# williamfgc/ROCm-MPI

Measured on AMD Instinct MI355X. Metric: T_eff (GB/s) + weak-scaling eff., 2D diffusion 1000 steps at 1/2/4/8 MI355X, higher is better.
Workload: dtype fp64

## Files before the change

csrc/bindings/module.cpp:

```cpp
#include <pybind11/pybind11.h>
#include <pybind11/stl.h>

#include <cstdint>
#include <string>
#include <tuple>
#include <vector>

#include "rma/config.h"
#include "rma/comm.h"
#include "rma/common.h"
#include "rma/executor.h"
#include "rma/gather.h"
#include "rma/halo.h"
#include "rma/ipc.h"
#include "rma/kernels.h"
#include "rma/loopback.h"
#include "rma/p2p.h"
#include "rma/plan.h"
#include "rma/topology.h"
#include "rma/trace.h"

namespace py = pybind11;
using namespace rma;

namespace {

template <typename T>
T* P(uintptr_t p) {
  return reinterpret_cast<T*>(p);
}
stream_t S(uintptr_t s) { return reinterpret_cast<stream_t>(s); }

using Rect4 = std::tuple<int64_t, int64_t, int64_t, int64_t>;
using Coef4 = std::tuple<double, double, double, double>;
using Geom = std::tuple<int64_t, int64_t, int64_t, int64_t, double, double, double, double, int,
                        int>;

std::vector<Rect> to_rects(const std::vector<Rect4>& v) {
  std::vector<Rect> r;
  for (auto& t : v) r.push_back({std::get<0>(t), std::get<1>(t), std::get<2>(t), std::get<3>(t)});
  return r;
}
StencilCoef to_coef(const Coef4& c) {
  return {std::get<0>(c), std::get<1>(c), std::get<2>(c), std::get<3>(c)};
}
TileGeom to_geom(const Geom& g) {
  TileGeom t;
  std::tie(t.gx0, t.gy0, t.nxg, t.nyg, t.dx, t.dy, t.xoff, t.yoff, t.periodx, t.periody) = g;
  return t;
}
Rect4 from_rect(const Rect& r) { return {r.x0, r.x1, r.y0, r.y1}; }

using Box6 = std::tuple<int64_t, int64_t, int64_t, int64_t, int64_t, int64_t>;
using Coef5 = std::tuple<double, double, double, double, double>;
using Geom3 = std::tuple<int64_t, int64_t, int64_t, int64_t, int64_t, int64_t, double, double,
                         double, double, double, double, int, int,
                         int>;
std::vector<Box> to_boxes(const std::vector<Box6>& v) {
  std::vector<Box> b;
  for (auto& t : v)
    b.push_back({std::get<0>(t), std::get<1>(t), std::get<2>(t), std::get<3>(t), std::get<4>(t),
                 std::get<5>(t)});
  return b;
}
StencilCoef3 to_coef3(const Coef5& c) {
  return {std::get<0>(c), std::get<1>(c), std::get<2>(c), std::get<3>(c), std::get<4>(c)};
}
TileGeom3 to_geom3(const Geom3& g) {
  TileGeom3 t;
  std::tie(t.gx0, t.gy0, t.gz0, t.nxg, t.nyg, t.nzg, t.dx, t.dy, t.dz, t.xoff, t.yoff, t.zoff,
           t.periodx, t.periody, t.periodz) = g;
  return t;
}

using FieldT = std::tuple<uintptr_t, std::array<int64_t, 3>, int, std::array<int64_t, 3>,
                          std::array<int64_t, 3>>;
std::vector<HaloField> to_fields(const std::vector<FieldT>& v) {
  std::vector<HaloField> out;
  for (auto& t : v) {
    HaloField f;
    f.ptr = reinterpret_cast<void*>(std::get<0>(t));
    f.size = std::get<1>(t);
    f.elem_bytes = std::get<2>(t);
    f.ol = std::get<3>(t);
    f.hw = std::get<4>(t);
    out.push_back(f);
  }
  return out;
}

}

PYBIND11_MODULE(_C, m) {
  m.doc() = "rocm_mpi_amd native core (HIP kernels for gfx950, RCCL halo exchange, executor)";
  static py::exception<Error> exc(m, "NativeError", PyExc_RuntimeError);
  py::register_exception_translator([](std::exception_ptr p) {
    try {
      if (p) std::rethrow_exception(p);
    } catch (const Error& e) {
      exc(e.what());
    }
  });

  m.def("set_rank_for_errors", &set_rank_for_errors);
  m.def("rccl_version", &rccl_version);
  m.def("rccl_library", &rccl_library);
  m.def("device_pci_bus_id", &device_pci_bus_id, py::arg("device"));
  m.def(
      "stencil_strip_cells",
      [](int64_t nx, int vec) {
        StencilTuning t;
        t.vec = vec;
        return stencil_strip_cells(nx, t);
      },
      py::arg("nx"), py::arg("vec") = 2);

  m.def(
      "stencil_rects",
      [](uintptr_t T2, uintptr_t T, uintptr_t iCp, int64_t nx, int64_t ny,
         const std::vector<Rect4>& rects, const Coef4& coef, int chunk_rows, int nontemporal,
         int kernel, uintptr_t stream, bool gpu, int unroll, int vec, int xcd_remap) {
        auto r = to_rects(rects);
        StencilTuning tn;
        tn.chunk_rows = chunk_rows;
        tn.nontemporal = nontemporal;
        tn.kernel = kernel;
        tn.unroll = unroll;
        tn.vec = vec;
        tn.xcd_remap = xcd_remap;
        if (gpu)
          stencil_rects_gpu(P<double>(T2), P<const double>(T), P<const double>(iCp), nx, ny,
                            r.data(), (int)r.size(), to_coef(coef), tn, S(stream));
        else {
          py::gil_scoped_release nogil;
          stencil_rects_cpu(P<double>(T2), P<const double>(T), P<const double>(iCp), nx, ny,
                            r.data(), (int)r.size(), to_coef(coef));
        }
      },
      py::arg("T2"), py::arg("T"), py::arg("iCp"), py::arg("nx"), py::arg("ny"), py::arg("rects"),
      py::arg("coef"), py::arg("chunk_rows") = 4, py::arg("nontemporal") = 3,
      py::arg("kernel") = 0, py::arg("stream") = 0, py::arg("gpu") = true,
      py::arg("unroll") = 4, py::arg("vec") = 2, py::arg("xcd_remap") = -1);
  m.def(
      "stencil2_rects",
      [](uintptr_t T2, uintptr_t T, uintptr_t iCp, int64_t nx, int64_t ny,
         const std::vector<Rect4>& rects, const Coef4& coef, int chunk_rows, int nontemporal,
         uintptr_t stream, bool gpu, int unroll, int xcd_remap) {
        auto r = to_rects(rects);
        StencilTuning tn;
        tn.chunk_rows = chunk_rows;
        tn.nontemporal = nontemporal;
        tn.unroll = unroll;
        tn.xcd_remap = xcd_remap;
        if (gpu)
          stencil2_rects_gpu(P<double>(T2), P<const double>(T), P<const double>(iCp), nx, ny,
                             r.data(), (int)r.size(), to_coef(coef), tn, S(stream));
        else {
          py::gil_scoped_release nogil;
          stencil2_rects_cpu(P<double>(T2), P<const double>(T), P<const double>(iCp), nx, ny,
                             r.data(), (int)r.size(), to_coef(coef));
        }
      },
      py::arg("T2"), py::arg("T"), py::arg("iCp"), py::arg("nx"), py::arg("ny"), py::arg("rects"),
      py::arg("coef"), py::arg("chunk_rows") = 8, py::arg("nontemporal") = 3,
      py::arg("stream") = 0, py::arg("gpu") = true, py::arg("unroll") = 2,
      py::arg("xcd_remap") = -1);
  m.def(
      "stencilk_rects",
      [](int K, uintptr_t T2, uintptr_t T, uintptr_t iCp, int64_t nx, int64_t ny,
         const std::vector<Rect4>& rects, const Coef4& coef, int chunk_rows, int nontemporal,
         uintptr_t stream, bool gpu, int xcd_remap, int vec, int kernel, int stages, int cols,
         bool uniform, double uniform_value) {
        auto r = to_rects(rects);
        StencilTuning tn;
        tn.cols = cols;
        tn.uniform = uniform;
        tn.uniform_value = uniform_value;
        tn.chunk_rows = chunk_rows;
        tn.nontemporal = nontemporal;
        tn.xcd_remap = xcd_remap;
        tn.vec = vec;
        tn.kernel = kernel;
        tn.stages = stages;
        if (gpu)
          stencilk_rects_gpu(K, P<double>(T2), P<const double>(T), P<const double>(iCp), nx, ny,
                             r.data(), (int)r.size(), to_coef(coef), tn, S(stream));
        else {
          const bool f5 = (kernel >= 5 && kernel <= 9) || kernel == 12 || kernel == 22;
          py::gil_scoped_release nogil;
          if (f5)
            stencilk5_rects_cpu(K, P<double>(T2), P<const double>(T), P<const double>(iCp), nx,
                                ny, r.data(), (int)r.size(), to_coef(coef));
          else
            stencilk_rects_cpu(K, P<double>(T2), P<const double>(T), P<const double>(iCp), nx,
                               ny, r.data(), (int)r.size(), to_coef(coef));
        }
      },
      py::arg("K"), py::arg("T2"), py::arg("T"), py::arg("iCp"), py::arg("nx"), py::arg("ny"),
      py::arg("rects"), py::arg("coef"), py::arg("chunk_rows") = 16, py::arg("nontemporal") = 3,
      py::arg("stream") = 0, py::arg("gpu") = true, py::arg("xcd_remap") = -1,
      py::arg("vec") = 2, py::arg("kernel") = 0, py::arg("stages") = 0, py::arg("cols") = 0,
      py::arg("uniform") = false, py::arg("uniform_value") = 0.0);
  m.def(
      "stencil3d_boxes",
      [](uintptr_t T2, uintptr_t T, uintptr_t iCp, int64_t nx, int64_t ny, int64_t nz,
         const std::vector<Box6>& boxes, const Coef5& coef, int rows, int unroll, int vec,
         int nontemporal, int chunk_z, int xcd_remap, uintptr_t stream, bool gpu) {
        auto b = to_boxes(boxes);
        if (gpu) {
          Stencil3DTuning tn;
          tn.rows = rows;
          tn.unroll = unroll;
          tn.vec = vec;
          tn.nontemporal = nontemporal;
          tn.chunk_z = chunk_z;
          tn.xcd_remap = xcd_remap;
          stencil3d_boxes_gpu(P<double>(T2), P<const double>(T), P<const double>(iCp), nx, ny, nz,
                              b.data(), (int)b.size(), to_coef3(coef), tn, S(stream));
        } else {
          py::gil_scoped_release nogil;
          stencil3d_boxes_cpu(P<double>(T2), P<const double>(T), P<const double>(iCp), nx, ny, nz,
                              b.data(), (int)b.size(), to_coef3(coef));
        }
      },
      py::arg("T2"), py::arg("T"), py::arg("iCp"), py::arg("nx"), py::arg("ny"), py::arg("nz"),
      py::arg("boxes"), py::arg("coef"), py::arg("rows") = 4, py::arg("unroll") = 2,
      py::arg("vec") = 2, py::arg("nontemporal") = 3, py::arg("chunk_z") = 0,
      py::arg("xcd_remap") = 1, py::arg("stream") = 0, py::arg("gpu") = true);
  m.def("stencil3d_has", &stencil3d_has, py::arg("rows"), py::arg("unroll"));
  m.def("init_gaussian3d", [](uintptr_t T, int64_t nx, int64_t ny, int64_t nz, const Geom3& g,
                              double lx, double ly, double lz, uintptr_t stream, bool gpu) {
    if (gpu)
      init_gaussian3d_gpu(P<double>(T), nx, ny, nz, to_geom3(g), lx, ly, lz, S(stream));
    else
      init_gaussian3d_cpu(P<double>(T), nx, ny, nz, to_geom3(g), lx, ly, lz);
  });
  m.def("init_random3d", [](uintptr_t A, int64_t nx, int64_t ny, int64_t nz, const Geom3& g,
                            uint64_t seed, double lo, double hi, uintptr_t stream, bool gpu) {
    if (gpu)
      init_random3d_gpu(P<double>(A), nx, ny, nz, to_geom3(g), seed, lo, hi, S(stream));
    else
      init_random3d_cpu(P<double>(A), nx, ny, nz, to_geom3(g), seed, lo, hi);
  });
  m.def(
      "stream_copy",
      [](uintptr_t b, uintptr_t a, int64_t n, uintptr_t s, int nt, int blocks) {
        stream_copy_gpu(P<double>(b), P<const double>(a), n, nt, blocks, S(s));
      },
      py::arg("b"), py::arg("a"), py::arg("n"), py::arg("stream"), py::arg("nt") = 0,
      py::arg("blocks") = 0);
  m.def(
      "stream_triad",
      [](uintptr_t c, uintptr_t a, uintptr_t b, double x, int64_t n, uintptr_t s, int nt,
         int blocks) {
        stream_triad_gpu(P<double>(c), P<const double>(a), P<const double>(b), x, n, nt, blocks,
                         S(s));
      },
      py::arg("c"), py::arg("a"), py::arg("b"), py::arg("x"), py::arg("n"), py::arg("stream"),
      py::arg("nt") = 0, py::arg("blocks") = 0);

  m.def("flux", [](uintptr_t qx, uintptr_t qy, uintptr_t T, int64_t nx, int64_t ny, double mlam,
                   double rdx, double rdy, uintptr_t stream, bool gpu) {
    if (gpu)
      flux_gpu(P<double>(qx), P<double>(qy), P<const double>(T), nx, ny, mlam, rdx, rdy,
               S(stream));
    else
      flux_cpu(P<double>(qx), P<double>(qy), P<const double>(T), nx, ny, mlam, rdx, rdy);
  });
  m.def("residual", [](uintptr_t dTdt, uintptr_t qx, uintptr_t qy, uintptr_t iCp, int64_t nx,
                       int64_t ny, double rdx, double rdy, uintptr_t stream, bool gpu) {
    if (gpu)
      residual_gpu(P<double>(dTdt), P<const double>(qx), P<const double>(qy),
                   P<const double>(iCp), nx, ny, rdx, rdy, S(stream));
    else
      residual_cpu(P<double>(dTdt), P<const double>(qx), P<const double>(qy),
                   P<const double>(iCp), nx, ny, rdx, rdy);
  });
  m.def("update", [](uintptr_t T, uintptr_t dTdt, int64_t nx, int64_t ny, double dt,
                     uintptr_t stream, bool gpu) {
    if (gpu)
      update_gpu(P<double>(T), P<const double>(dTdt), nx, ny, dt, S(stream));
    else
      update_cpu(P<double>(T), P<const double>(dTdt), nx, ny, dt);
  });
  m.def("init_gaussian", [](uintptr_t T, int64_t nx, int64_t ny, const Geom& g, double lx,
                            double ly, uintptr_t stream, bool gpu) {
    if (gpu)
      init_gaussian_gpu(P<double>(T), nx, ny, to_geom(g), lx, ly, S(stream));
    else
      init_gaussian_cpu(P<double>(T), nx, ny, to_geom(g), lx, ly);
  });
  m.def("init_random", [](uintptr_t A, int64_t nx, int64_t ny, const Geom& g, uint64_t seed,
                          double lo, double hi, uintptr_t stream, bool gpu) {
    if (gpu)
      init_random_gpu(P<double>(A), nx, ny, to_geom(g), seed, lo, hi, S(stream));
    else
      init_random_cpu(P<double>(A), nx, ny, to_geom(g), seed, lo, hi);
  });
  m.def("fill", [](uintptr_t A, int64_t n, double v, uintptr_t stream) {
    fill_gpu(P<double>(A), n, v, S(stream));
  });
  m.def("copy2d", [](uintptr_t dst, int64_t dst_ld, uintptr_t src, int64_t src_ld, int64_t n_o,
                     int64_t n_k, int elem_bytes, uintptr_t stream, bool gpu) {
    if (gpu)
      copy2d_gpu(P<void>(dst), dst_ld, P<const void>(src), src_ld, n_o, n_k, elem_bytes,
                 S(stream));
    else
      copy2d_cpu(P<void>(dst), dst_ld, P<const void>(src), src_ld, n_o, n_k, elem_bytes);
  });
  m.def("copy2d_batch", [](const std::vector<std::tuple<uintptr_t, int64_t, uintptr_t, int64_t,
                                                        int64_t, int64_t>>& copies,
                           int elem_bytes, uintptr_t stream, bool gpu) {
    std::vector<Copy2d> c;
    for (const auto& t : copies)
      c.push_back({P<void>(std::get<0>(t)), std::get<1>(t), P<const void>(std::get<2>(t)),
                   std::get<3>(t), std::get<4>(t), std::get<5>(t)});
    if (gpu)
      copy2d_batch_gpu(c.data(), (int)c.size(), elem_bytes, S(stream));
    else
      copy2d_batch_cpu(c.data(), (int)c.size(), elem_bytes);
  });
  m.def("copy2d_batch_max", [] { return kCopy2dBatch; });
  m.def("copy_blocks", [](const std::vector<std::tuple<uintptr_t, uintptr_t, int64_t, int64_t,
                                                       int64_t, int64_t, int64_t, int64_t,
                                                       int64_t>>& blocks,
                          int elem_bytes, uintptr_t stream, bool gpu) {
    std::vector<BlockCopy> c;
    for (const auto& t : blocks)
      c.push_back({P<void>(std::get<0>(t)), P<const void>(std::get<1>(t)), std::get<2>(t),
                   std::get<3>(t), std::get<4>(t), std::get<5>(t), std::get<6>(t),
                   std::get<7>(t), std::get<8>(t)});
    if (gpu)
      copy_blocks_gpu(c.data(), (int64_t)c.size(), elem_bytes, S(stream));
    else
      copy_blocks_cpu(c.data(), (int64_t)c.size(), elem_bytes);
  });
  m.def("copy_blocks_max", [] { return kCopyBlocksBatch; });
  m.def(
      "gather_plan",
      [](const std::array<int, 3>& dims, const std::array<int64_t, 3>& size, int elem_bytes) {
        const GatherPlan p = plan_gather(dims, size, elem_bytes);
        py::dict d;
        d["nprocs"] = p.nprocs;
        d["size_g"] = p.size_g;
        d["row_pitch_g"] = p.row_pitch_g;
        d["plane_pitch_g"] = p.plane_pitch_g;
        d["block_elems"] = p.block_elems;
        d["coords"] = p.coords;
        d["offsets"] = p.offset;
        d["contiguous_in_global"] = p.contiguous_in_global;
        return d;
      },
      py::arg("dims"), py::arg("size"), py::arg("elem_bytes"));
  m.def(
      "flag_wait",
      [](uintptr_t flag, uint64_t want, double timeout_s, uintptr_t err, uint32_t code,
         uintptr_t stream) {
        flag_wait_gpu(P<const uint64_t>(flag), want, timeout_s, P<uint32_t>(err), code, S(stream));
      },
      py::call_guard<py::gil_scoped_release>());
  m.def(
      "flag_write",
      [](uintptr_t flag, uint64_t value, uintptr_t stream) {
        flag_write_gpu(P<uint64_t>(flag), value, S(stream));
      },
      py::call_guard<py::gil_scoped_release>());
  m.def("reduce_workspace_doubles", &reduce_workspace_doubles);
  m.def("reduce_gpu", [](uintptr_t A, int64_t n, int op, uintptr_t out, uintptr_t ws,
                         uintptr_t stream) {
    reduce_gpu(P<const double>(A), n, op, P<double>(out), P<double>(ws), S(stream));
  });
  m.def("reduce_cpu",
        [](uintptr_t A, int64_t n, int op) { return reduce_cpu(P<const double>(A), n, op); });
  m.def("diag_string", &diag_string);
  m.def("diag_value", [](const std::string& k) { return diag_value(k.c_str()); });
  m.def("env_double", &env_double);
  m.def("env_choice", &env_choice);
  m.def("field_stats_workspace_doubles", &field_stats_workspace_doubles);
  m.def("field_stats_gpu", [](uintptr_t A, int64_t n, uintptr_t out3, uintptr_t ws,
                              uintptr_t stream) {
    field_stats_gpu(P<const double>(A), n, P<double>(out3), P<double>(ws), S(stream));
  });
  m.def("field_stats_cpu", [](uintptr_t A, int64_t n) {
    double o[3];
    field_stats_cpu(P<const double>(A), n, o);
    return std::make_tuple(o[0], o[1], o[2]);
  });

  m.def("dims_create", &dims_create, py::arg("nprocs"), py::arg("dims"));
  m.attr("PROC_NULL") = kProcNull;
  py::class_<CartTopology>(m, "CartTopology")
      .def(py::init<int, std::array<int, 3>, std::array<int, 3>>(), py::arg("nprocs"),
           py::arg("dims"), py::arg("periods"))
      .def_property_readonly("nprocs", &CartTopology::nprocs)
      .def_property_readonly("dims", &CartTopology::dims)
      .def_property_readonly("periods", &CartTopology::periods)
      .def("coords", &CartTopology::coords)
      .def("rank_of", &CartTopology::rank_of)
      .def("shift", &CartTopology::shift)
      .def("neighbors", &CartTopology::neighbors)
      .def("diagonals", &CartTopology::diagonals);

  py::enum_<DType>(m, "DType")
      .value("float64", DType::kFloat64)
      .value("float32", DType::kFloat32)
      .value("int64", DType::kInt64)
      .value("int32", DType::kInt32)
      .value("uint8", DType::kUInt8);
  py::enum_<RedOp>(m, "RedOp")
      .value("sum", RedOp::kSum)
      .value("max", RedOp::kMax)
      .value("min", RedOp::kMin)
      .value("prod", RedOp::kProd);
  py::class_<P2PTransport>(m, "P2PTransport")
      .def_property_readonly("rank", &P2PTransport::rank)
      .def_property_readonly("size", &P2PTransport::size)
      .def("group_start", &P2PTransport::group_start)
      .def("group_end", &P2PTransport::group_end, py::call_guard<py::gil_scoped_release>())
      .def("send", [](P2PTransport& c, uintptr_t buf, size_t bytes, int peer,
                      uintptr_t s) { c.send(P<const void>(buf), bytes, peer, S(s)); },
           py::call_guard<py::gil_scoped_release>())
      .def("recv", [](P2PTransport& c, uintptr_t buf, size_t bytes, int peer,
                      uintptr_t s) { c.recv(P<void>(buf), bytes, peer, S(s)); },
           py::call_guard<py::gil_scoped_release>());
  py::class_<LoopbackHub, std::shared_ptr<LoopbackHub>>(m, "LoopbackHub")
      .def(py::init<int, double>(), py::arg("nranks"), py::arg("timeout_s") = 60.0)
      .def_property_readonly("size", &LoopbackHub::size);
  py::class_<LoopbackEndpoint, P2PTransport>(m, "LoopbackEndpoint")
      .def(py::init<std::shared_ptr<LoopbackHub>, int>(), py::arg("hub"), py::arg("rank"));
  py::class_<IpcTransport, P2PTransport>(m, "IpcTransport")
      .def(py::init<int, int, int, const std::vector<int>&, size_t, const std::string&, double,
                    int>(),
           py::arg("rank"), py::arg("size"), py::arg("device"), py::arg("peers"),
           py::arg("mailbox_bytes"), py::arg("token"), py::arg("timeout_s") = 300.0,
           py::arg("mode") = -1)
      .def("export_for", [](const IpcTransport& t, int p) { return py::bytes(t.export_for(p)); })
      .def("connect", [](IpcTransport& t, int p, py::bytes blob) { t.connect(p, blob); })
      .def("unlink_shm", &IpcTransport::unlink_shm)
      .def("abort_waits", &IpcTransport::abort_waits)
      .def("check_error", &IpcTransport::check_error)
      .def_property_readonly("connected", &IpcTransport::connected)
      .def_property_readonly("mailbox_bytes", &IpcTransport::mailbox_bytes)
      .def_property_readonly("mode",
                             [](const IpcTransport& t) {
                               return t.mode() == IpcTransport::Mode::kStream ? "stream" : "host";
                             })
      .def_property_readonly("poisoned", &IpcTransport::poisoned)
      .def_property_readonly("host_waits", &IpcTransport::host_waits);
  py::class_<IpcMap>(m, "IpcMap")
      .def(py::init<>())
      .def_static("export_ptr",
                  [](uintptr_t p) { return py::bytes(IpcMap::export_ptr((const void*)p)); })
      .def("open", [](IpcMap& m, py::bytes blob) { return (uintptr_t)m.open(blob); })
      .def("close_all", &IpcMap::close_all)
      .def_property_readonly("mappings", &IpcMap::mappings);
  py::class_<RcclComm, P2PTransport>(m, "RcclComm")
      .def_static("unique_id", []() { return py::bytes(RcclComm::unique_id()); })
      .def(py::init([](int nranks, int rank, py::bytes uid, int device, double init_timeout_s) {
             std::string s = uid;
             py::gil_scoped_release nogil;
             return new RcclComm(nranks, rank, s, device, init_timeout_s);
           }),
           py::arg("nranks"), py::arg("rank"), py::arg("uid"), py::arg("device"),
           py::arg("init_timeout_s") = 0.0)
      .def_property_readonly("nonblocking", &RcclComm::nonblocking)
      .def_property_readonly("data_blocking", &RcclComm::data_blocking)
      .def_property_readonly("device", &RcclComm::device)
      .def("count", &RcclComm::count)
      .def("allreduce",
           [](RcclComm& c, uintptr_t sb, uintptr_t rb, size_t count, DType dt, RedOp op,
              uintptr_t s) { c.allreduce(P<const void>(sb), P<void>(rb), count, dt, op, S(s)); })
      .def("broadcast",
           [](RcclComm& c, uintptr_t sb, uintptr_t rb, size_t count, DType dt, int root,
              uintptr_t s) { c.broadcast(P<const void>(sb), P<void>(rb), count, dt, root, S(s)); })
      .def("gather", [](RcclComm& c, uintptr_t sb, uintptr_t rb, size_t bytes, int root,
                        uintptr_t s) { c.gather(P<const void>(sb), P<void>(rb), bytes, root, S(s)); })
      .def(
          "barrier", [](RcclComm& c, uintptr_t s, double t) { c.barrier(S(s), t); },
          py::arg("stream"), py::arg("timeout_s") = 300.0, py::call_guard<py::gil_scoped_release>())
      .def(
          "wait", [](RcclComm& c, uintptr_t s, double t) { c.wait(S(s), t); }, py::arg("stream"),
          py::arg("timeout_s") = 300.0, py::call_guard<py::gil_scoped_release>())
      .def("check_async", &RcclComm::check_async)
      .def("abort", &RcclComm::abort)
      .def_property_readonly("aborted", &RcclComm::aborted);

  py::class_<HaloExchanger>(m, "HaloExchanger")
      .def(py::init([](P2PTransport* comm, int self_rank,
                       std::array<std::array<int, 2>, 3> nbr) {
             return new HaloExchanger(comm, self_rank, nbr);
           }),
           py::arg("comm").none(true), py::arg("self_rank"), py::arg("neighbors"),
           py::keep_alive<1, 2>())
      .def(
          "exchange",
          [](HaloExchanger& h, const std::vector<FieldT>& fields, uintptr_t s, int mask) {
            auto f = to_fields(fields);
            py::gil_scoped_release nogil;
            h.exchange(f, S(s), mask);
          },
          py::arg("fields"), py::arg("stream"), py::arg("dims_mask") = 7)
      .def(
          "prepare",
          [](HaloExchanger& h, const std::vector<FieldT>& fields, int mask) {
            h.prepare(to_fields(fields), mask);
          },
          py::arg("fields"), py::arg("dims_mask") = 7)
      .def(
          "exchange_merged",
          [](HaloExchanger& h, const std::vector<FieldT>& fields, uintptr_t s) {
            auto f = to_fields(fields);
            py::gil_scoped_release nogil;
            h.exchange_merged(f, S(s));
          },
          py::arg("fields"), py::arg("stream"))
      .def("set_diagonals", &HaloExchanger::set_diagonals)
      .def_property_readonly("has_diagonals", &HaloExchanger::has_diagonals)
      .def_property_readonly("diagonals", &HaloExchanger::diagonals)
      .def("active", &HaloExchanger::active)
      .def("capturable", &HaloExchanger::capturable)
      .def("set_self_via_transport", &HaloExchanger::set_self_via_transport)
      .def_property_readonly("neighbors", &HaloExchanger::neighbors)
      .def_property_readonly("bytes_sent_last", &HaloExchanger::bytes_sent_last)
      .def_property_readonly("plan_hits", &HaloExchanger::plan_hits)
      .def_property_readonly("plan_misses", &HaloExchanger::plan_misses);

  m.def("pipe_chunk_rows", &pipe_chunk_rows, py::arg("K"), py::arg("ny"),
        py::arg("canonical") = false);
  m.def("default_chunk_k", [](int K, int64_t ny) { return default_tune_k(K, ny).chunk_rows; },
        py::arg("K"), py::arg("ny"));
  m.def("plan_passes", &plan_passes, py::arg("nsteps"), py::arg("costs"));
  m.def("default_pass_costs", &default_pass_costs, py::arg("kmax"), py::arg("fast5"),
        py::arg("cells") = 0.0);
  m.def("pipe_default_stages", &pipe_default_stages, py::arg("K"));
  m.def("pipe_default_cols", &pipe_default_cols, py::arg("K"), py::arg("stages"),
        py::arg("arith") = 0);
  m.def("pipe_has_cols", &pipe_has_cols, py::arg("K"), py::arg("stages"), py::arg("arith"),
        py::arg("cols"));
  m.def("pipe_vec", &pipe_vec, py::arg("K"), py::arg("stages"), py::arg("arith"), py::arg("nx"),
        py::arg("requested"), py::arg("aligned16") = true);
  m.def("pipe_max_k", []() { return kPipeMaxK; });
  m.def(
      "pass_geometry",
      [](int64_t nx, int64_t ny, int K, std::array<std::array<int, 2>, 3> nbr, bool hide,
         int64_t bwx, int64_t bwy, int64_t olx, int64_t oly) {
        const PassGeom g = pass_geometry(nx, ny, K, nbr, hide, bwx, bwy, olx, oly);
        std::vector<Rect4> fr;
        for (auto& r : g.frame) fr.push_back(from_rect(r));
        return std::make_tuple(from_rect(g.out), fr, from_rect(g.interior));
      },
      py::arg("nx"), py::arg("ny"), py::arg("K"), py::arg("neighbors"), py::arg("hide"),
      py::arg("bwx"), py::arg("bwy"), py::arg("olx"), py::arg("oly"));
  m.def(
      "frame_layout",
      [](int64_t ny, std::array<std::array<int, 2>, 3> nbr) {
        const FrameLayout f = frame_layout(ny, nbr);
        return std::make_tuple(f.chunk_div, f.bands);
      },
      py::arg("ny"), py::arg("neighbors"));
  m.def(
      "canonical_kernel_k",
      [](int K, int64_t ny) {
        const StencilTuning t = canonical_tune_k(K, ny);
        return std::make_tuple(t.kernel, t.vec, t.chunk_rows);
      },
      py::arg("K"), py::arg("ny"));
  m.def(
      "fast_kernel_k",
      [](int K, int64_t ny, const Coef4& coef) {
        const StencilTuning t = fast_tune_k(K, ny, to_coef(coef));
        return std::make_tuple(t.kernel, t.vec, t.chunk_rows);
      },
      py::arg("K"), py::arg("ny"), py::arg("coef"));
  py::class_<DiffusionExecutor>(m, "Executor")
      .def(py::init([](uintptr_t T, uintptr_t T2, uintptr_t iCp, int64_t nx, int64_t ny, int mode,
                       const Coef4& coef, int chunk_rows, int nontemporal, int kernel,
                       int64_t bwx, int64_t bwy, int use_graph, int graph_steps,
                       HaloExchanger* halo, uintptr_t qx, uintptr_t qy, uintptr_t dTdt,
                       int unroll, int vec, int temporal, int64_t olx, int64_t oly,
                       int chunk2, int unroll2, int fast_math) {
             ExecParams p;
             p.fast_math = fast_math;
             p.temporal = temporal;
             p.olx = olx;
             p.oly = oly;
             p.tune2 = default_tune_k(temporal, ny);
             if (chunk2 > 0) p.tune2.chunk_rows = chunk2;
             p.chunk_rows2 = chunk2;
             if (temporal == 2) p.tune2.unroll = unroll2;
             p.tune2.nontemporal = nontemporal & 3;
             p.mode = static_cast<Mode>(mode);
             p.coef = to_coef(coef);
             p.tune.chunk_rows = chunk_rows;
             p.tune.nontemporal = nontemporal;
             p.tune.kernel = kernel;
             p.tune.unroll = unroll;
             p.tune.vec = vec;
             p.bwx = bwx;
             p.bwy = bwy;
             p.use_graph = use_graph;
             p.graph_steps = graph_steps;
             return new DiffusionExecutor(P<double>(T), P<double>(T2), P<const double>(iCp), nx,
                                          ny, p, halo, P<double>(qx), P<double>(qy),
                                          P<double>(dTdt));
           }),
           py::arg("T"), py::arg("T2"), py::arg("iCp"), py::arg("nx"), py::arg("ny"),
           py::arg("mode"), py::arg("coef"), py::arg("chunk_rows") = 4,
           py::arg("nontemporal") = 3, py::arg("kernel") = 0, py::arg("bwx") = 1,
           py::arg("bwy") = 1, py::arg("use_graph") = 0, py::arg("graph_steps") = 0,
           py::arg("halo").none(true) = nullptr, py::arg("qx") = 0, py::arg("qy") = 0,
           py::arg("dTdt") = 0, py::arg("unroll") = 4, py::arg("vec") = 2,
           py::arg("temporal") = 1, py::arg("olx") = 2, py::arg("oly") = 2,
           py::arg("chunk2") = 0, py::arg("unroll2") = 2, py::arg("fast_math") = 0,
           py::keep_alive<1, 16>())
      .def(
          "run", [](DiffusionExecutor& e, int64_t n, uintptr_t s) { e.run(n, S(s)); },
          py::arg("nsteps"), py::arg("stream"), py::call_guard<py::gil_scoped_release>())
      .def_property_readonly("parity", &DiffusionExecutor::parity)
      .def_property_readonly("steps_done", &DiffusionExecutor::steps_done)
      .def_property_readonly("passes_done", &DiffusionExecutor::passes_done)
      .def_property_readonly("fused_passes", &DiffusionExecutor::fused_passes)
      .def_property_readonly("uniform_factor", &DiffusionExecutor::uniform_factor)
      .def("rescan_factor", &DiffusionExecutor::rescan_factor,
           py::call_guard<py::gil_scoped_release>())
      .def("check_error", &DiffusionExecutor::check_error)
      .def("plan", &DiffusionExecutor::plan, py::arg("nsteps"))
      .def_property_readonly("pass_costs", &DiffusionExecutor::pass_costs)
      .def("prime", &DiffusionExecutor::prime, py::call_guard<py::gil_scoped_release>())
      .def("set_timing", &DiffusionExecutor::set_timing, py::arg("on"),
           py::call_guard<py::gil_scoped_release>())
      .def("timings",
           [](DiffusionExecutor& e) {
             std::vector<py::dict> out;
             std::vector<PassTiming> ts;
             {
               py::gil_scoped_release nogil;
               ts = e.timings();
             }
             for (const auto& t : ts) {
               py::dict d;
               d["K"] = t.K;
               d["frame_ms"] = t.frame_ms;
               d["halo_ms"] = t.halo_ms;
               d["interior_ms"] = t.interior_ms;
               d["pass_ms"] = t.pass_ms;
               d["exposed_halo_ms"] = t.exposed_halo_ms;
               out.push_back(d);
             }
             return out;
           })
      .def(
          "set_direct",
          [](DiffusionExecutor& e, const std::vector<std::tuple<int, uintptr_t, uintptr_t, uintptr_t>>& peers,
             uintptr_t in_flags, bool host_wait) {
            RMA_CHECK_ARG(peers.size() == 8, "set_direct: 8 directions, got " << peers.size());
            std::array<DiffusionExecutor::DirectPeer, 8> a{};
            for (int d = 0; d < 8; ++d) {
              a[d].rank = std::get<0>(peers[d]);
              a[d].T = P<double>(std::get<1>(peers[d]));
              a[d].T2 = P<double>(std::get<2>(peers[d]));
              a[d].flag = P<uint64_t>(std::get<3>(peers[d]));
            }
            e.set_direct(a, P<uint64_t>(in_flags), host_wait);
          },
          py::arg("peers"), py::arg("in_flags"), py::arg("host_wait") = false,
          py::call_guard<py::gil_scoped_release>())
      .def_property_readonly("direct", &DiffusionExecutor::direct)
      .def_property_readonly("direct_passes", &DiffusionExecutor::direct_passes)
      .def_property_readonly_static("direct_dirs", [](py::object) {
        std::vector<std::pair<int, int>> v;
        for (int d = 0; d < 8; ++d)
          v.emplace_back(DiffusionExecutor::kDirI[d], DiffusionExecutor::kDirJ[d]);
        return v;
      })
      .def("set_solo", &DiffusionExecutor::set_solo, py::arg("on"),
           py::call_guard<py::gil_scoped_release>())
      .def_property_readonly("solo", &DiffusionExecutor::solo)
      .def_property_readonly("frame_rects",
                             [](const DiffusionExecutor& e) {
                               std::vector<Rect4> v;
                               for (auto& r : e.frame_rects()) v.push_back(from_rect(r));
                               return v;
                             })
      .def_property_readonly("interior_rect",
                             [](const DiffusionExecutor& e) { return from_rect(e.interior_rect()); })
      .def(
          "geometry",
          [](DiffusionExecutor& e, int K) {
            const PassGeom& g = e.geometry(K);
            auto rl = [](const std::vector<Rect>& v) {
              std::vector<Rect4> o;
              for (auto& r : v) o.push_back(from_rect(r));
              return o;
            };
            py::dict d;
            d["aligned"] = g.aligned;
            d["out"] = from_rect(g.out);
            d["frame"] = rl(g.frame);
            d["frame_wide"] = rl(g.frame_wide);
            d["frame_tall"] = rl(g.frame_tall);
            d["interior"] = from_rect(g.interior);
            d["tasks"] = g.tasks();
            return d;
          },
          py::arg("K"));

  m.def("trace_enable", &trace_enable);
  m.def("trace_enabled", &trace_enabled);
  m.def("trace_push", [](const std::string& s) { trace_push(s.c_str()); });
  m.def("trace_pop", &trace_pop);
  m.def("trace_mark", [](const std::string& s) { trace_mark(s.c_str()); });
}
```

csrc/include/rma/executor.h:

```cpp
#pragma once

#include <array>
#include <cstdint>
#include <memory>
#include <vector>

#include "rma/halo.h"
#include "rma/kernels.h"
#include "rma/plan.h"

namespace rma {

enum class Mode : int { kPerf = 0, kHide = 1, kKp = 2 };

struct ExecParams {
  Mode mode = Mode::kPerf;
  StencilCoef coef{};
  StencilTuning tune{};
  int64_t bwx = 1, bwy = 1;
  int use_graph = 0;
  int graph_steps = 0;
  int temporal = 1;
  int64_t olx = 2, oly = 2;
  StencilTuning tune2{16, 3, 0, 2, 2, -1};
  int chunk_rows2 = 0;
  int fast_math = 0;
};

StencilTuning default_tune_k(int K, int64_t ny);
StencilTuning fast_tune_k(int K, int64_t ny, const StencilCoef& c);
StencilTuning canonical_tune_k(int K, int64_t ny);

struct PassTiming {
  int K = 0;
  float frame_ms = 0, halo_ms = 0, interior_ms = 0, pass_ms = 0, exposed_halo_ms = 0;
};

class DiffusionExecutor {
 public:
  DiffusionExecutor(double* T, double* T2, const double* iCp, int64_t nx, int64_t ny,
                    const ExecParams& p, HaloExchanger* halo, double* qx = nullptr,
                    double* qy = nullptr, double* dTdt = nullptr);
  ~DiffusionExecutor();
  DiffusionExecutor(const DiffusionExecutor&) = delete;
  DiffusionExecutor& operator=(const DiffusionExecutor&) = delete;

  void run(int64_t nsteps, stream_t caller_stream);
  std::vector<int> plan(int64_t nsteps) const;
  const std::vector<double>& pass_costs() const { return cost_; }
  void prime();
  void set_timing(bool on);
  std::vector<PassTiming> timings();
  void set_solo(bool on);
  bool solo() const { return solo_; }
  int parity() const { return parity_; }
  int64_t steps_done() const { return steps_; }
  int64_t passes_done() const { return passes_; }
  int64_t fused_passes() const { return fused_passes_; }
  void check_error() const { check_fused_error(); }
  bool uniform_factor() const { return uniform_; }
  bool rescan_factor();
  struct DirectPeer {
    int rank = -1;
    double* T = nullptr;
    double* T2 = nullptr;
    uint64_t* flag = nullptr;
  };
  static constexpr int kDirI[8] = {-1, 0, 1, -1, 1, -1, 0, 1};
  static constexpr int kDirJ[8] = {-1, -1, -1, 0, 0, 1, 1, 1};
  void set_direct(const std::array<DirectPeer, 8>& peers, uint64_t* in_flags,
                  bool host_wait = false);
  bool direct() const { return direct_on_; }
  int64_t direct_passes() const { return direct_pass_; }
  std::vector<Rect> frame_rects() const { return frame_; }
  Rect interior_rect() const { return interior_; }
  Rect full_rect() const { return full_; }
  const PassGeom& geometry(int K);

 private:
  void enqueue_step(double* Tin, double* Tout);
  void enqueue_pass(int K, double* Tin, double* Tout);
  StencilTuning pass_tuning(int K, int part = 0) const;
  int frame_chunk_rows(int K, int interior_rows) const;
  void multi_step(int K, double* Tin, double* Tout, const double* iCp, int64_t nx, int64_t ny,
                  const Rect* rects, int n, const StencilTuning& tn, void* stream) const;
  void exchange(double* A, stream_t s);
  bool cross_pass_ = false;
  void build_graph(int64_t steps, int reps);
  void run_eager(int64_t nsteps);
  bool fast5() const;
  void scan_factor();
  bool uniform_ = false;
  double c0_ = 0.0;

  double* T_;
  double* T2_;
  const double* iCp_;
  int64_t nx_, ny_;
  ExecParams p_;
  HaloExchanger* halo_;
  double *qx_, *qy_, *dTdt_;
  Neighbors nbr_{{{-1, -1}, {-1, -1}, {-1, -1}}};
  Rect full_{}, interior_{};
  std::vector<Rect> frame_;
  std::vector<PassGeom> geom_;
  std::vector<char> geom_ok_;
  std::vector<double> cost_;
  std::vector<double> cost_base_;
  int64_t hwx_ = 1, hwy_ = 1;
  void* s_hi_ = nullptr;
  void* s_lo_ = nullptr;
  void* e_hi_ = nullptr;
  void* e_lo_ = nullptr;
  void* e_in_ = nullptr;
  void* e_fr_ = nullptr;
  bool lag_ = true;
  int fused_ = 2;
  int cus_ = 256;
  int64_t fused_passes_ = 0;
  double fused_timeout_s_ = 60.0;
  uint64_t* sig_ = nullptr;
  uint32_t* ferr_host_ = nullptr;
  uint32_t* ferr_dev_ = nullptr;
  bool fused_pass_ok(const PassGeom& g, const StencilTuning& tn) const;
  template <typename Launch>
  void enqueue_fused(const std::vector<Rect>& frame, const Rect& interior, StencilTuning tn,
                     double* Tout, void* const* ev, Launch&& launch);
  void check_fused_error() const;
  bool direct_on_ = false;
  std::array<DirectPeer, 8> dpeer_{};
  uint64_t* din_flags_ = nullptr;
  uint32_t din_mask_ = 0;
  FlagTargets dout_{};
  uint64_t direct_pass_ = 0;
  bool dhost_ = false;
  void direct_wait(uint64_t want, void* stream);
  bool direct_active() const { return direct_on_ && !solo_; }
  bool direct_remote() const { return direct_active() && din_mask_ != 0; }
  DirectStores direct_stores(bool out_is_T2) const;
  bool images_in_frame(const PassGeom& g) const;
  DirectStores dstores_[2];
  void ensure_error_word();
  void* graph_exec_ = nullptr;
  int64_t graph_len_ = 0;
  int parity_ = 0;
  int64_t steps_ = 0;
  int64_t passes_ = 0;
  bool solo_ = false;
  bool pooled_ = false;
  Neighbors real_nbr_{{{-1, -1}, {-1, -1}, {-1, -1}}};
  bool timing_ = false;
  std::vector<void*> tev_;
  std::vector<int> tk_;
  std::vector<char> tseq_;
  size_t tused_ = 0;
  void* tevent();
  void release_timing();
  void release_resources();
};

}
```

csrc/include/rma/kernels.h:

```cpp
#pragma once

#include <cstddef>
#include <cstdint>

#include "rma/common.h"

namespace rma {

using stream_t = void*;

constexpr int kMaxRects = 8;

struct DirectStores {
  int on = 0;
  int32_t xm0 = 0, xm1 = 0, xp0 = 0, xp1 = 0;
  int32_t ym0 = 0, ym1 = 0, yp0 = 0, yp1 = 0;
  int64_t sx = 0, syr = 0;
  double* dst[8] = {};
};

struct StencilTuning {
  int chunk_rows = 4;
  int nontemporal = 3;
  int kernel = 0;
  int unroll = 4;
  int vec = 2;
  int xcd_remap = -1;
  int stages = 0;
  int cols = 0;
  uint64_t* signal = nullptr;
  int signal_rects = 0;
  int signal_chunk_rows = 0;
  const DirectStores* direct = nullptr;
  bool uniform = false;
  double uniform_value = 0.0;
};

void stencil_rects_gpu(double* T2, const double* T, const double* iCp, int64_t nx, int64_t ny,
                       const Rect* rects, int nrects, const StencilCoef& c,
                       const StencilTuning& tune, stream_t stream);
void stencil_rects_cpu(double* T2, const double* T, const double* iCp, int64_t nx, int64_t ny,
                       const Rect* rects, int nrects, const StencilCoef& c);

void stencil2_rects_gpu(double* T2, const double* T, const double* iCp, int64_t nx, int64_t ny,
                        const Rect* rects, int nrects, const StencilCoef& c,
                        const StencilTuning& tune, stream_t stream);
void stencil2_rects_cpu(double* T2, const double* T, const double* iCp, int64_t nx, int64_t ny,
                        const Rect* rects, int nrects, const StencilCoef& c);

void stencilk_rects_gpu(int K, double* T2, const double* T, const double* iCp, int64_t nx,
                        int64_t ny, const Rect* rects, int nrects, const StencilCoef& c,
                        const StencilTuning& tune, stream_t stream);
void stencilk_rects_cpu(int K, double* T2, const double* T, const double* iCp, int64_t nx,
                        int64_t ny, const Rect* rects, int nrects, const StencilCoef& c);
bool fast5_ok(const StencilCoef& c);
constexpr int kPipeMaxK = 24;
int pipe_default_stages(int K);
bool pipe_has(int K, int stages, int arith = 0);
bool pipe_has_cols(int K, int stages, int arith, int cols);
int pipe_default_cols(int K, int stages, int arith);
int pipe_vec(int K, int stages, int arith, int64_t nx, int requested, bool aligned16);
void stencil_pipe_occupancy(int K, int stages, int arith, int V, int occ[2]);
void stencil_pipe_rects_gpu(int K, int stages, int arith, double* T2, const double* T,
                            const double* iCp, int64_t nx, int64_t ny, const Rect* rects,
                            int nrects, const StencilCoef& c, const StencilTuning& tune,
                            stream_t stream);
void stencil5_rects_cpu(double* T2, const double* T, const double* iCp, int64_t nx, int64_t ny,
                        const Rect* rects, int nrects, const StencilCoef& c);
void stencilk5_rects_cpu(int K, double* T2, const double* T, const double* iCp, int64_t nx,
                         int64_t ny, const Rect* rects, int nrects, const StencilCoef& c);

void count_differing_gpu(const double* A, int64_t n, uint64_t* out2, stream_t stream);
int64_t count_differing_cpu(const double* A, int64_t n);

constexpr int kMaxBoxes = 8;

struct Stencil3DTuning {
  int rows = 4;
  int unroll = 2;
  int vec = 2;
  int nontemporal = 3;
  int chunk_z = 0;
  int xcd_remap = 1;
};
bool stencil3d_has(int rows, int unroll);

void stencil3d_boxes_gpu(double* T2, const double* T, const double* iCp, int64_t nx, int64_t ny,
                         int64_t nz, const Box* boxes, int nboxes, const StencilCoef3& c,
                         const Stencil3DTuning& tune, stream_t stream);
void stencil3d_boxes_cpu(double* T2, const double* T, const double* iCp, int64_t nx, int64_t ny,
                         int64_t nz, const Box* boxes, int nboxes, const StencilCoef3& c);
void validate_boxes(const double* T2, const double* T, int64_t nx, int64_t ny, int64_t nz,
                    const Box* boxes, int nboxes);

int stencil_vec(int64_t nx, const StencilTuning& tune);
int stencil_strip_cells(int64_t nx, const StencilTuning& tune);

void flux_gpu(double* QX, double* QY, const double* T, int64_t nx, int64_t ny, double mlam,
              double rdx, double rdy, stream_t stream);
void residual_gpu(double* D, const double* QX, const double* QY, const double* iCp, int64_t nx,
                  int64_t ny, double rdx, double rdy, stream_t stream);
void update_gpu(double* T, const double* D, int64_t nx, int64_t ny, double dt, stream_t stream);
void flux_cpu(double* QX, double* QY, const double* T, int64_t nx, int64_t ny, double mlam,
              double rdx, double rdy);
void residual_cpu(double* D, const double* QX, const double* QY, const double* iCp, int64_t nx,
                  int64_t ny, double rdx, double rdy);
void update_cpu(double* T, const double* D, int64_t nx, int64_t ny, double dt);
bool kp_native_layout_ok(int64_t nx);

struct TileGeom {
  int64_t gx0, gy0;
  int64_t nxg, nyg;
  double dx, dy;
  double xoff, yoff;
  int periodx, periody;
};

void init_gaussian_gpu(double* T, int64_t nx, int64_t ny, const TileGeom& g, double lx, double ly,
                       stream_t stream);
void init_gaussian_cpu(double* T, int64_t nx, int64_t ny, const TileGeom& g, double lx, double ly);
void init_random_gpu(double* A, int64_t nx, int64_t ny, const TileGeom& g, uint64_t seed,
                     double lo, double hi, stream_t stream);
void init_random_cpu(double* A, int64_t nx, int64_t ny, const TileGeom& g, uint64_t seed,
                     double lo, double hi);
void fill_gpu(double* A, int64_t n, double value, stream_t stream);

struct TileGeom3 {
  int64_t gx0, gy0, gz0;
  int64_t nxg, nyg, nzg;
  double dx, dy, dz;
  double xoff, yoff, zoff;
  int periodx, periody, periodz;
};
void init_gaussian3d_gpu(double* T, int64_t nx, int64_t ny, int64_t nz, const TileGeom3& g,
                         double lx, double ly, double lz, stream_t stream);
void init_gaussian3d_cpu(double* T, int64_t nx, int64_t ny, int64_t nz, const TileGeom3& g,
                         double lx, double ly, double lz);
void init_random3d_gpu(double* A, int64_t nx, int64_t ny, int64_t nz, const TileGeom3& g,
                       uint64_t seed, double lo, double hi, stream_t stream);
void init_random3d_cpu(double* A, int64_t nx, int64_t ny, int64_t nz, const TileGeom3& g,
                       uint64_t seed, double lo, double hi);

void copy2d_gpu(void* dst, int64_t dst_ld, const void* src, int64_t src_ld, int64_t n_o,
                int64_t n_k, int elem_bytes, stream_t stream);
void copy2d_cpu(void* dst, int64_t dst_ld, const void* src, int64_t src_ld, int64_t n_o,
                int64_t n_k, int elem_bytes);
constexpr int kCopy2dBatch = 8;
struct Copy2d {
  void* dst;
  int64_t dst_ld;
  const void* src;
  int64_t src_ld, n_o, n_k;
};
void copy2d_batch_gpu(const Copy2d* copies, int n, int elem_bytes, stream_t stream);
void copy2d_batch_cpu(const Copy2d* copies, int n, int elem_bytes);

struct BlockCopy {
  void* dst;
  const void* src;
  int64_t dst_row, dst_plane, src_row, src_plane;
  int64_t nx, ny, nz;
};
constexpr int kCopyBlocksBatch = 32;
void validate_block_copies(const BlockCopy* blocks, int64_t n, int elem_bytes);
void copy_blocks_gpu(const BlockCopy* blocks, int64_t n, int elem_bytes, stream_t stream);
void copy_blocks_cpu(const BlockCopy* blocks, int64_t n, int elem_bytes);

void stream_copy_gpu(double* b, const double* a, int64_t n, int nt, int blocks, stream_t stream);
void stream_triad_gpu(double* c, const double* a, const double* b, double s, int64_t n, int nt,
                      int blocks, stream_t stream);

void flag_wait_gpu(const uint64_t* flag, uint64_t want, double timeout_s, uint32_t* err,
                   uint32_t code, stream_t stream);
void flag_write_gpu(uint64_t* flag, uint64_t value, stream_t stream);
void flags_wait_ge_gpu(const uint64_t* flags, uint32_t mask, uint64_t want, double timeout_s,
                       uint32_t* err, uint32_t code, stream_t stream);
struct FlagTargets {
  uint64_t* dst[8] = {};
};
void flags_write_gpu(const FlagTargets& t, uint64_t value, stream_t stream);

enum ReduceOp : int { kSum = 0, kMax = 1, kMin = 2, kMaxAbs = 3, kNonFinite = 4 };
int64_t reduce_workspace_doubles();
void reduce_gpu(const double* A, int64_t n, int op, double* out, double* workspace,
                stream_t stream);
double reduce_cpu(const double* A, int64_t n, int op);
int64_t field_stats_workspace_doubles();
void field_stats_gpu(const double* A, int64_t n, double* out3, double* workspace,
                     stream_t stream);
void field_stats_cpu(const double* A, int64_t n, double* out3);

}
```

csrc/include/rma/plan.h:

```cpp
#pragma once

#include <array>
#include <cstdint>
#include <vector>

#include "rma/common.h"

namespace rma {

using Neighbors = std::array<std::array<int, 2>, 3>;

void split_rect(const Rect& out, int64_t bwx, int64_t bwy, std::vector<Rect>& frame,
                Rect& interior);
void split_rect_sides(const Rect& out, int64_t xlo, int64_t xhi, int64_t ylo, int64_t yhi,
                      std::vector<Rect>& frame, Rect& interior);

Rect owned_rect(int64_t nx, int64_t ny, int K, const Neighbors& nbr);

std::array<std::array<bool, 2>, 2> frame_sides(const Neighbors& nbr);

struct PassGeom {
  Rect out{};
  std::vector<Rect> frame;
  Rect interior{};
  std::vector<Rect> frame_wide, frame_tall;
  bool aligned = false;
  int64_t task_w = 0, task_h = 0;
  int64_t tasks() const {
    if (task_w <= 0 || task_h <= 0 || out.empty()) return 0;
    return ((out.x1 - out.x0 + task_w - 1) / task_w) * ((out.y1 - out.y0 + task_h - 1) / task_h);
  }
};

PassGeom pass_geometry(int64_t nx, int64_t ny, int K, const Neighbors& nbr, bool hide,
                       int64_t bwx, int64_t bwy, int64_t olx, int64_t oly, int64_t task_w = 0,
                       int64_t task_h = 0, int vec = 1, int bands = -1, int out_k = 0);

struct FrameLayout {
  int chunk_div = 1;
  int bands = -1;
};
FrameLayout frame_layout(int64_t ny, const Neighbors& nbr);

std::vector<double> default_pass_costs(int kmax, bool fast5, double cells = 0);
void apply_cost_overrides(std::vector<double>& cost, const char* spec);

int pipe_chunk_rows(int K, int64_t ny, bool canonical);

std::vector<int> plan_passes(int64_t n, const std::vector<double>& cost);

}
```

csrc/kernels/kernel_select.cpp:

```cpp
#include <cstdint>

#include "pipe_arith.h"
#include "rma/kernels.h"

namespace rma {

int pipe_default_stages(int K) {
  if (K <= 4) return 1;
  if (K <= 9) return 2;
  return 4;
}

bool pipe_has(int K, int S, int arith) {
  if (K < 1 || K > kPipeMaxK) return false;
  if (arith == pipe::kArFast5Reg) return S == 4 && K >= 10 && K <= 24;
  if (arith == pipe::kArFast5RegNoSB) return S == 4 && (K == 20 || K == 24);
  if (arith != pipe::kArFast5 && arith != pipe::kArCanon) return false;
  if (S == pipe_default_stages(K)) return true;
  return (K == 12 && S == 3) || (K == 16 && S == 8) || (K == 24 && S == 8) ||
         (K == 8 && S == 4) || (K == 8 && S == 1);
}

bool pipe_has_cols(int K, int S, int arith, int cols) {
  if (cols <= 1) return pipe_has(K, S, arith);
  if (cols != 2 || S != 4) return false;
  return (arith == pipe::kArFast5 || arith == pipe::kArFast5Reg) && (K == 16 || K == 20 || K == 24);
}

int pipe_default_cols(int K, int S, int arith) {
  (void)K;
  (void)S;
  (void)arith;
  return 1;
}

int pipe_vec(int K, int stages, int arith, int64_t nx, int requested, bool aligned16) {
  const int S = stages > 0 ? stages : pipe_default_stages(K);
  if (requested == 5 && nx % 5 == 0 && pipe::pipe_has_v5(K, S, arith)) return 5;
  if (aligned16 && nx % 2 == 0) return (requested >= 4 && nx % 4 == 0) ? 4 : 2;
  return 1;
}

int stencil_vec(int64_t nx, const StencilTuning& tune) {
  if (nx % 2) return 1;
  if (tune.vec == 4 && nx % 4 == 0) return 4;
  return 2;
}

int stencil_strip_cells(int64_t nx, const StencilTuning& tune) {
  constexpr int kWave = 64;
  return kWave * stencil_vec(nx, tune);
}

}
```

csrc/kernels/pipe_arith.h:

```cpp
#pragma once

namespace rma {
namespace pipe {

constexpr int kArFast5 = 0, kArCanon = 1, kArFast5Reg = 3, kArFast5RegNoSB = 13;
constexpr bool ar_reg(int Ar) { return Ar == kArFast5Reg || Ar == kArFast5RegNoSB; }

inline bool pipe_has_v5(int K, int S, int ar) {
  return ar == kArFast5 && S == 4 && K >= 16 && K <= 20;
}

}
}
```

csrc/kernels/stencil_pipe.h:

```cpp
#pragma once

#include <hip/hip_runtime.h>

#include <type_traits>

#include "pipe_arith.h"
#include "rma/common.h"
#include "rma/hip_check.h"
#include "rma/kernels.h"
#include "stencil_device.h"

namespace rma {
namespace pipe {
using namespace march;

template <int K, int S>
struct Plan {
  static constexpr int H = (K + S - 1) / S;
  static constexpr int HL = K - (S - 1) * H;
  static constexpr int R = K + S - 1;
  static_assert(S >= 1 && HL >= 1 && HL <= H, "bad stage split");
};

template <int V>
constexpr bool kDelayedRing = V == 5;
template <int K, int S, int V>
constexpr int ring_rows() {
  return Plan<K, S>::R - (kDelayedRing<V> ? 1 : 0);
}

template <int K, int S, int V, int C>
struct Geo {
  static constexpr int W = kWave * V;
  static constexpr int Hp = (Plan<K, S>::H + 1) / 2 * 2;
  static constexpr int D = C > 1 ? W - 2 * Hp : W;
  static constexpr int WB = (C - 1) * D + W;
  static constexpr int kStep = (WB - 2 * K) / V * V;
  static_assert(C == 1 || (V == 4 && D % 4 == 0 && D > 2 * K / S), "bad column split");
};


template <int K, int S, int V, bool Canon, int C = 1>
constexpr int occupancy(int lds) {
  const int by_lds = (160 * 1024) / lds * S * C / 4;
  const int vgpr = Canon ? 8 * Plan<K, S>::H * V + 8 * V + 64
                         : (V == 5 ? 5 : 6) * Plan<K, S>::H * V + 8 * V + 40;
  const int by_vgpr = 512 / ((vgpr + 7) / 8 * 8);
  const int w = by_lds < by_vgpr ? by_lds : by_vgpr;
  return w < 1 ? 1 : (w > 8 ? 8 : w);
}

template <int K, int S, int V, bool Canon, int C = 1>
constexpr int mirror_rows() {
  constexpr int H = Plan<K, S>::H, row = Geo<K, S, V, C>::WB * 8;
  constexpr int base = (ring_rows<K, S, V>() + 2 * (S > 1 ? S - 1 : 1)) * row;
  return occupancy<K, S, V, Canon, C>(base + (H - 1) * row) ==
                 occupancy<K, S, V, Canon, C>(base)
             ? H - 1
             : 0;
}

template <int K, int S, int V, bool Canon, int C = 1>
constexpr int lds_bytes() {
  return (ring_rows<K, S, V>() + mirror_rows<K, S, V, Canon, C>() + 2 * (S > 1 ? S - 1 : 1)) *
         Geo<K, S, V, C>::WB * 8;
}

template <int K, int S, int V, bool Canon, int C = 1>
constexpr int waves_per_simd() {
  return occupancy<K, S, V, Canon, C>(lds_bytes<K, S, V, Canon, C>());
}

template <int K, int S, int Ar, bool Uni = false>
constexpr bool pipe_u6() {
  return ar_reg(Ar) && !Uni && Plan<K, S>::H == 5;
}
template <int K, int S, int Ar, bool Uni = false>
constexpr int staging_rows() {
  return pipe_u6<K, S, Ar, Uni>() ? 6 : 3;
}
template <int K, int S, int V, int Ar, int C = 1, bool Uni = false>
constexpr int lds_bytes_reg() {
  return ((Uni ? 2 : 4) * (S > 1 ? S - 1 : 1) * Geo<K, S, V, C>::WB +
          (V == 2 || V == 4
               ? (Uni ? 1 : 2) * staging_rows<K, S, Ar, Uni>() * Geo<K, S, V, C>::W * C
               : 0)) *
             8 +
         8;
}
template <int K, int S, int V, int Ar, int C, bool Uni = false>
constexpr int kernel_waves() {
  if constexpr (ar_reg(Ar)) {
    constexpr int H = Plan<K, S>::H;
    constexpr int vgpr = (Uni ? 6 : 8) * H * V + 8 * V + 40;
    constexpr int by_vgpr = 512 / ((vgpr + 7) / 8 * 8);
    constexpr int w = occupancy<K, S, V, false, C>(lds_bytes_reg<K, S, V, Ar, C, Uni>());
    return by_vgpr < 2 ? 2 : (by_vgpr < w ? by_vgpr : w);
  } else {
    return waves_per_simd<K, S, V, Ar == kArCanon, C>();
  }
}

__device__ __forceinline__ double from_next_lane(double v) {
  const int lo = __builtin_amdgcn_mov_dpp(__double2loint(v), 0x130, 0xf, 0xf, true);
  const int hi = __builtin_amdgcn_mov_dpp(__double2hiint(v), 0x130, 0xf, 0xf, true);
  return __hiloint2double(hi, lo);
}
__device__ __forceinline__ double from_prev_lane(double v) {
  const int lo = __builtin_amdgcn_mov_dpp(__double2loint(v), 0x138, 0xf, 0xf, true);
  const int hi = __builtin_amdgcn_mov_dpp(__double2hiint(v), 0x138, 0xf, 0xf, true);
  return __hiloint2double(hi, lo);
}

template <int V>
__device__ __forceinline__ void direct_row(const DirectStores& D, int row, int64_t nx, int x32,
                                           int64_t e, const double (&res)[V],
                                           const bool (&m)[V], bool dxm, bool dxp) {
  const bool ym = row >= D.ym0 && row < D.ym1, yp = row >= D.yp0 && row < D.yp1;
  const int64_t sx = D.sx, sy = D.syr * nx;
  auto put = [&](int d, int64_t off, const bool (&mk)[V]) {
    if (D.dst[d]) store_row<V, true>(D.dst[d] + (e + off), res, mk);
  };
  if (ym) put(1, sy, m);
  if (yp) put(6, -sy, m);
  auto xside = [&](int dx, int dd0, int dd1, int64_t ox, int32_t a0, int32_t a1) {
    bool mk[V];
#pragma unroll
    for (int v = 0; v < V; ++v) mk[v] = m[v] && x32 + v >= a0 && x32 + v < a1;
    put(dx, ox, mk);
    if (ym) put(dd0, ox + sy, mk);
    if (yp) put(dd1, ox - sy, mk);
  };
  if (dxm) xside(3, 0, 5, sx, D.xm0, D.xm1);
  if (dxp) xside(4, 2, 7, -sx, D.xp0, D.xp1);
}

template <int K, int S, int V, int Ar, int C, bool Dir, bool Uni>
__device__ __forceinline__ void pipe_body(double* __restrict__ T2, const double* __restrict__ T,
                                          const double* __restrict__ iCp, int64_t nx, int64_t ny,
                                          const RectList& L, const StencilCoef& k, int chunk_rows,
                                          int remap, const DirectStores& DS, double c0) {
  using P = Plan<K, S>;
  constexpr bool Canon = Ar == kArCanon, kRegG = ar_reg(Ar);
  static_assert(!kRegG || (V != 5 && (C == 1 || V == 4)),
                "register factors: V <= 4; two column waves at V = 4 only");
  constexpr bool kGlds = kRegG && (V == 2 || V == 4);
  static_assert(!Uni || (kGlds && C == 1 && !Dir),
                "uniform factor: register factors, 2 or 4 cells per lane, one column wave, "
                "no direct stores");
  constexpr bool kU6 = pipe_u6<K, S, Ar, Uni>();
  constexpr int NST = staging_rows<K, S, Ar, Uni>();
  using G = Geo<K, S, V, C>;
  constexpr int H = P::H, HL = P::HL, R = ring_rows<K, S, V>();
  constexpr int M = kRegG ? 0 : mirror_rows<K, S, V, Canon, C>();
  constexpr bool kDelay = kDelayedRing<V>;
  static_assert(V != 5 || (C == 1 && Ar == kArFast5), "5 cells per lane: fast5, one column wave");
  constexpr int W = G::W, WB = G::WB, D = G::D;
  constexpr int kStep = G::kStep;
  constexpr int NH = S > 1 ? S - 1 : 1;
  const int wv = __builtin_amdgcn_readfirstlane(threadIdx.x >> 6);
  const int col = C > 1 ? wv / S : 0;
  const int stage = wv % S;
  const int lane = threadIdx.x & (kWave - 1);
  const int64_t sig_first = L.sig ? L.sig_blocks : 0;
  const int64_t b = remap ? xcd_remap_after(blockIdx.x, gridDim.x, sig_first) : (int64_t)blockIdx.x;
  int ri = 0;
  while (ri < L.n - 1 && b >= L.block_end[ri]) ++ri;
  const int64_t lb = b - (ri ? L.block_end[ri - 1] : 0);
  const int64_t strip = lb % L.strips[ri], chunk = lb / L.strips[ri];
  const Rect r = L.r[ri];
  const int64_t xs = L.xa[ri] + strip * kStep;
  const int64_t crows = L.crows[ri];
  const int64_t ya = r.y0 + chunk * crows;
  const int64_t yb = min(r.y1, ya + crows);

  const int lo = col > 0 ? G::Hp : 0, hi = col < C - 1 ? D + G::Hp : W;
  const int64_t xw = xs + (int64_t)col * D;
  const int64_t x = xw + (int64_t)lane * V;
  bool m[V], cin[V];
#pragma unroll
  for (int v = 0; v < V; ++v) {
    const int p = lane * V + v, pb = col * D + p;
    m[v] = pb >= K && pb < K + kStep && p >= lo && p < hi && x + v >= r.x0 && x + v < r.x1;
    cin[v] = (x + v >= 1) && (x + v <= nx - 2);
  }
  const int64_t xl = min(max(x, (int64_t)0), nx - V);
  const uint32_t xo = (uint32_t)xl, xso = (uint32_t)x;
  const uint32_t xob = xo * 8u, xsob = xso * 8u;
  auto at = [](const double* base, uint32_t boff) {
    return reinterpret_cast<const double*>(reinterpret_cast<const char*>(base) + boff);
  };
  const bool xin = xw >= 1 && xw + W - 1 <= nx - 2;
  bool dxm = false, dxp = false, dtask = false;
  if constexpr (Dir) {
    bool pm = false, pp = false;
#pragma unroll
    for (int v = 0; v < V; ++v) {
      pm = pm || (m[v] && x + v >= DS.xm0 && x + v < DS.xm1);
      pp = pp || (m[v] && x + v >= DS.xp0 && x + v < DS.xp1);
    }
    dxm = __builtin_amdgcn_ballot_w64(pm) != 0;
    dxp = __builtin_amdgcn_ballot_w64(pp) != 0;
    const bool tym = ya < DS.ym1 && yb > DS.ym0, typ = ya < DS.yp1 && yb > DS.yp0;
    dtask = dxm || dxp || tym || typ;
  }

  const double ax = (-k.mlam) * k.rdx * k.rdx;
  const double ay = (-k.mlam) * k.rdy * k.rdy;
  const double ry = Canon ? 0.0 : ay / ax;
  const double mkc = -2.0 * (1.0 + ry);
  const double gs = Canon ? 1.0 : k.dt * ax;

  double w[H][3][V], fy[Canon ? H : 1][V], pT[V], pC[V], qT[V], qC[V];
#pragma unroll
  for (int j = 0; j < H; ++j)
#pragma unroll
    for (int v = 0; v < V; ++v) {
      w[j][0][v] = w[j][1][v] = w[j][2][v] = 0.0;
      fy[Canon ? j : 0][v] = 0.0;
    }
  const int ny32 = (int)ny, ya32 = (int)ya, yb32 = (int)yb;
  int i = ya32 - K;
  const int iend = yb32 + K - 3 + S;
  auto rowc = [&](int y) { return (int64_t)min(max(y, 0), ny32 - 1); };
  auto rowp = [&](const double* a, int y) { return at(a + rowc(y) * nx, xob); };
  if (stage == 0) {
    load_row<V>(w[0][2], rowp(T, i));
    if constexpr (!kGlds) {
      load_row<V>(pT, rowp(T, i + 1));
      load_row<V>(pC, rowp(iCp, i));
      load_row<V>(qT, rowp(T, i + 2));
      load_row<V>(qC, rowp(iCp, i + 1));
    }
  }
  constexpr int kRing = kRegG ? 1 : (R + M) * WB, kHand = kRegG && !Uni ? 4 : 2;
  constexpr int kStgArrays = Uni ? 1 : 2;
  __shared__ double ring[kRing];
  __shared__ double hand[kHand][NH][WB];
  __shared__ double staging[kGlds ? kStgArrays * NST * W * C : 1];
  if constexpr (!kRegG)
    for (int t = threadIdx.x; t < kRing; t += S * C * kWave) ring[t] = 0.0;
  for (int t = threadIdx.x; t < kHand * NH * WB; t += S * C * kWave) (&hand[0][0][0])[t] = 0.0;
  constexpr int NG = kRegG && !Uni ? H : 1;
  double gr[NG][V];
#pragma unroll
  for (int q = 0; q < NG; ++q)
#pragma unroll
    for (int v = 0; v < V; ++v) gr[q][v] = 0.0;
  auto gh = [&](int pb, int st) { return &hand[(kHand - 2) + pb][st][0]; };
  auto gshift = [&]() {
#pragma unroll
    for (int q = NG - 1; q > 0; --q)
#pragma unroll
      for (int v = 0; v < V; ++v) gr[q][v] = gr[q - 1][v];
  };
  __syncthreads();
  auto stg = [&](int a, int r) { return &staging[((kStgArrays * col + a) * NST + r) * W]; };
  auto glds_row = [&](int a, int y, int r) {
    const double* rb = (a ? iCp : T) + rowc(y) * nx;
#pragma unroll
    for (int h = 0; h < V / 2; ++h)
      __builtin_amdgcn_global_load_lds(at(rb, xob + 16u * h), stg(a, r) + h * 2 * kWave, 16, 0, 0);
  };
  if constexpr (kGlds) {
    if (stage == 0) {
#pragma unroll
      for (int r = 0; r < NST; ++r) {
        glds_row(0, i + 1 + r, r);
        if constexpr (!Uni) glds_row(1, i + r, r);
      }
    }
  }
  constexpr int NPH = V == 4 ? WB / 4 : kWave;
  const int cq = col * (D / 4);
  auto rd2 = [&](const double* row, double (&out)[V]) {
    if constexpr (V == 1) {
      out[0] = row[lane];
    } else if constexpr (V == 5) {
#pragma unroll
      for (int v = 0; v < V; ++v) out[v] = row[v * kWave + lane];
    } else {
#pragma unroll
      for (int h = 0; h < V / 2; ++h) {
        const dbl2 t2 = reinterpret_cast<const dbl2*>(row)[h * NPH + cq + lane];
        out[2 * h] = t2.x;
        out[2 * h + 1] = t2.y;
      }
    }
  };
  auto rds = [&](const double* row, double (&out)[V]) {
#pragma unroll
    for (int h = 0; h < V / 2; ++h) {
      const dbl2 t2 = reinterpret_cast<const dbl2*>(row)[h * kWave + lane];
      out[2 * h] = t2.x;
      out[2 * h + 1] = t2.y;
    }
  };
  auto wr2 = [&](double* row, const double (&in)[V]) {
    if constexpr (V == 1) {
      row[lane] = in[0];
    } else if constexpr (V == 5) {
#pragma unroll
      for (int v = 0; v < V; ++v) row[v * kWave + lane] = in[v];
    } else {
#pragma unroll
      for (int h = 0; h < V / 2; ++h) {
        dbl2 t2;
        t2.x = in[2 * h];
        t2.y = in[2 * h + 1];
        if (C == 1 || (lane * V + 2 * h >= lo && lane * V + 2 * h < hi))
          reinterpret_cast<dbl2*>(row)[h * NPH + cq + lane] = t2;
      }
    }
  };
  int slot0 = 0;
  double gp[V];
#pragma unroll
  for (int v = 0; v < V; ++v) gp[v] = 0.0;
  int par = 0;
  const int lag = stage * (H + 1);
  const double gU = gs * c0;
  const int gUlo = __builtin_amdgcn_readfirstlane(__double2loint(gU));
  const int gUhi = __builtin_amdgcn_readfirstlane(__double2hiint(gU));
  double gc[V];
#pragma unroll
  for (int v = 0; v < V; ++v) gc[v] = cin[v] ? gU : 0.0;

  auto iter = [&](auto Pc, auto S0c, auto LASTc, auto XINc) {
    constexpr bool XIN = decltype(XINc)::value;
    constexpr int Ps = decltype(Pc)::value;
    constexpr int Pr = Ps % 3;
    constexpr bool S0 = decltype(S0c)::value;
    constexpr bool LAST = decltype(LASTc)::value;
    constexpr int NL = LAST ? HL : H;
    constexpr int PC = (Pr + 2) % 3, PU = (Pr + 1) % 3;
    double g[V];
    if constexpr (S0) {
      if constexpr (kRegG && !Uni && !LAST) wr2(gh(par, 0), gr[NG - 1]);
      const bool rin1 = i >= 1 && i <= ny32 - 2;
      if constexpr (kGlds) {
        constexpr int kVm = (NST - 1) * kStgArrays * (V / 2);
        static_assert(kVm < 64, "vmcnt");
        __builtin_amdgcn_s_waitcnt(0x0F70 | (kVm & 15) | ((kVm >> 4) << 14));
        asm volatile("" ::: "memory");
        rds(stg(0, Ps), pT);
        if constexpr (!Uni) rds(stg(1, Ps), pC);
      }
#pragma unroll
      for (int v = 0; v < V; ++v) w[0][Pr][v] = pT[v];
      if constexpr (Uni) {
      } else if (rin1 && xin) {
#pragma unroll
        for (int v = 0; v < V; ++v) g[v] = Canon ? pC[v] : gs * pC[v];
      } else {
#pragma unroll
        for (int v = 0; v < V; ++v) g[v] = (rin1 && cin[v]) ? (Canon ? pC[v] : gs * pC[v]) : 0.0;
      }
      if constexpr (Uni) {
      } else if constexpr (kRegG) {
        gshift();
#pragma unroll
        for (int v = 0; v < V; ++v) gr[0][v] = g[v];
      } else if constexpr (kDelay) {
        const int sp = slot0 == 0 ? R - 1 : slot0 - 1;
        wr2(ring + (sp + M) * WB, gp);
        if constexpr (M > 0) {
          if (sp >= R - M) wr2(ring + (sp - (R - M)) * WB, gp);
        }
      } else {
        wr2(ring + (slot0 + M) * WB, g);
        if constexpr (M > 0) {
          if (slot0 >= R - M) wr2(ring + (slot0 - (R - M)) * WB, g);
        }
      }
      if constexpr (!kGlds) {
#pragma unroll
        for (int v = 0; v < V; ++v) {
          pT[v] = qT[v];
          pC[v] = qC[v];
        }
        load_row<V>(qT, rowp(T, i + 3));
        load_row<V>(qC, rowp(iCp, i + 2));
      }
    } else {
      rd2(&hand[par ^ 1][stage - 1][0], w[0][Pr]);
      if constexpr (kRegG && !Uni) {
        if constexpr (!LAST) wr2(gh(par, stage), gr[NG - 1]);
        gshift();
        rd2(gh(par ^ 1, stage - 1), gr[0]);
      }
    }
    int sbase = slot0 - (S0 ? 0 : lag);
    sbase = sbase < 0 ? sbase + R : sbase;
    const double* rbase = ring + (sbase + M) * WB;
    const double* rlow = ring + (sbase - (NL - 1)) * WB;
    auto levels = [&](auto NWc) {
    constexpr bool NW = decltype(NWc)::value;
    auto ring_row = [&](int j) {
      if constexpr (NW) {
        return rlow + (NL - j) * WB;
      } else if constexpr (M > 0) {
        return rbase - (j - 1) * WB;
      } else {
        const int sl = sbase - (j - 1) < 0 ? sbase - (j - 1) + R : sbase - (j - 1);
        return (const double*)(ring + sl * WB);
      }
    };
    auto fetch = [&](int j, double (&out)[V]) {
      if (S0 && kDelay && j == 2) {
#pragma unroll
        for (int v = 0; v < V; ++v) out[v] = gp[v];
      } else {
        rd2(ring_row(j), out);
      }
    };
    double gn[V];
    if constexpr (kRegG) {
    } else if constexpr (S0) {
#pragma unroll
      for (int v = 0; v < V; ++v) gn[v] = g[v];
    } else {
      rd2(ring_row(1), gn);
    }
#pragma unroll
    for (int j = 1; j <= NL; ++j) {
      const int row = i - (S0 ? 0 : lag) - (j - 1);
      double gl[V];
      if constexpr (Uni) {
        const bool rin = row >= 1 && row <= ny32 - 2;
        if constexpr (XIN) {
          const double gu = __hiloint2double(rin ? gUhi : 0, rin ? gUlo : 0);
#pragma unroll
          for (int v = 0; v < V; ++v) gl[v] = gu;
        } else {
#pragma unroll
          for (int v = 0; v < V; ++v) gl[v] = rin ? gc[v] : 0.0;
        }
      } else if constexpr (kRegG) {
#pragma unroll
        for (int v = 0; v < V; ++v) gl[v] = gr[j - 1][v];
      } else {
#pragma unroll
        for (int v = 0; v < V; ++v) gl[v] = gn[v];
        if (j < NL) fetch(j + 1, gn);
      }
      const double(&c)[V] = w[j - 1][PC];
      const double(&dn)[V] = w[j - 1][Pr];
      double res[V];
      if constexpr (!Canon) {
        const double(&up)[V] = w[j - 1][PU];
        const double rn = from_next_lane(c[0]);
        const double ln = from_prev_lane(c[V - 1]);
        double sx[V], sy[V], t[V];
#pragma unroll
        for (int v = 0; v < V; ++v) {
          const double rv = v + 1 < V ? c[v + 1] : rn;
          const double lv = v > 0 ? c[v - 1] : ln;
          sx[v] = rv + lv;
          sy[v] = up[v] + dn[v];
        }
        if constexpr (Ar != kArFast5RegNoSB) __builtin_amdgcn_sched_barrier(0);
#pragma unroll
        for (int v = 0; v < V; ++v) t[v] = __builtin_fma(mkc, c[v], sx[v]);
        if constexpr (Ar != kArFast5RegNoSB) __builtin_amdgcn_sched_barrier(0);
#pragma unroll
        for (int v = 0; v < V; ++v) t[v] = __builtin_fma(ry, sy[v], t[v]);
        if constexpr (Ar != kArFast5RegNoSB) __builtin_amdgcn_sched_barrier(0);
#pragma unroll
        for (int v = 0; v < V; ++v) res[v] = __builtin_fma(gl[v], t[v], c[v]);
      } else {
        const double rn = from_next_lane(c[0]);
        double qr[V];
#pragma unroll
        for (int v = 0; v < V; ++v) {
          const double rv = v + 1 < V ? c[v + 1] : rn;
          qr[v] = (k.mlam * (rv - c[v])) * k.rdx;
        }
        const double ql0 = from_prev_lane(qr[V - 1]);
#pragma unroll
        for (int v = 0; v < V; ++v) {
          const double qU = (k.mlam * (dn[v] - c[v])) * k.rdy;
          const double qD = fy[j - 1][v];
          fy[j - 1][v] = qU;
          const double qL = v == 0 ? ql0 : qr[v - 1];
          res[v] = c[v] + k.dt * (gl[v] * ((-(qr[v] - qL)) * k.rdx - (qU - qD) * k.rdy));
        }
      }
      if (j < NL) {
        const int jj = j < NL ? j : NL - 1;
#pragma unroll
        for (int v = 0; v < V; ++v) w[jj][Pr][v] = res[v];
      } else if constexpr (!LAST) {
        wr2(&hand[par][S0 ? 0 : stage][0], res);
      } else if (row >= ya32 && row < yb32) {
        store_row<V, true>(const_cast<double*>(at(T2 + (int64_t)row * nx, xsob)), res, m);
        if constexpr (Dir) {
          if (dtask)
            direct_row<V>(DS, row, nx, (int)xso, (int64_t)row * nx + x, res, m, dxm, dxp);
        }
      }
    }
    };
    if constexpr (M == 0 && kDelay) {
      if (sbase >= NL - 1)
        levels(std::true_type{});
      else
        levels(std::false_type{});
    } else {
      levels(std::false_type{});
    }
    if constexpr (S0 && kDelay) {
#pragma unroll
      for (int v = 0; v < V; ++v) gp[v] = g[v];
    }
    slot0 = slot0 + 1 == R ? 0 : slot0 + 1;
    par ^= 1;
    if constexpr (kGlds) {
      if constexpr (S0) {
        __builtin_amdgcn_s_waitcnt(0xC07F);
        asm volatile("" ::: "memory");
        glds_row(0, i + 1 + NST, Ps);
        if constexpr (!Uni) glds_row(1, i + NST, Ps);
      }
      asm volatile("s_waitcnt lgkmcnt(0)\n\ts_barrier" ::: "memory");
    } else {
      __syncthreads();
    }
  };
  auto run = [&](auto S0c, auto LASTc, auto XINc) {
    for (;;) {
      iter(std::integral_constant<int, 0>{}, S0c, LASTc, XINc);
      if (++i > iend) break;
      iter(std::integral_constant<int, 1>{}, S0c, LASTc, XINc);
      if (++i > iend) break;
      iter(std::integral_constant<int, 2>{}, S0c, LASTc, XINc);
      if (++i > iend) break;
      if constexpr (kU6) {
        iter(std::integral_constant<int, 3>{}, S0c, LASTc, XINc);
        if (++i > iend) break;
        iter(std::integral_constant<int, 4>{}, S0c, LASTc, XINc);
        if (++i > iend) break;
        iter(std::integral_constant<int, 5>{}, S0c, LASTc, XINc);
        if (++i > iend) break;
      }
    }
  };
  auto role = [&](auto XINc) {
    if constexpr (S == 1) {
      run(std::true_type{}, std::true_type{}, XINc);
    } else {
      if (stage == 0)
        run(std::true_type{}, std::false_type{}, XINc);
      else if (stage == S - 1)
        run(std::false_type{}, std::true_type{}, XINc);
      else if constexpr (S > 2)
        run(std::false_type{}, std::false_type{}, XINc);
    }
  };
  if constexpr (Uni) {
    if (xin)
      role(std::true_type{});
    else
      role(std::false_type{});
  } else {
    role(std::true_type{});
  }
  if constexpr (kGlds) {
    if (stage == 0) asm volatile("s_waitcnt vmcnt(0)" ::: "memory");
  }
  if (b < sig_first) signal_block_done(L.sig, L.sig_blocks);
}

template <int K, int S, int V, int Ar, int C, bool Dir = false, bool Uni = false>
__global__ __launch_bounds__(kWave * S * C) __attribute__((amdgpu_waves_per_eu(
    kernel_waves<K, S, V, Ar, C, Uni>()))) void pipe_kernel(double* __restrict__ T2,
                                                           const double* __restrict__ T,
                                                           const double* __restrict__ iCp,
                                                           int64_t nx, int64_t ny, RectList L,
                                                           StencilCoef k, int chunk_rows,
                                                           int remap, DirectStores D, double c0) {
  pipe_body<K, S, V, Ar, C, Dir, Uni>(T2, T, iCp, nx, ny, L, k, chunk_rows, remap, D, c0);
}

template <int V, int Ar, int C>
constexpr bool has_direct() {
  return C == 1 && V != 5 && (Ar == kArFast5 || Ar == kArFast5Reg || Ar == kArFast5RegNoSB);
}

template <int V, int Ar, int C>
constexpr bool has_uniform() {
  return C == 1 && (V == 2 || V == 4) && (Ar == kArFast5Reg || Ar == kArFast5RegNoSB);
}

struct PipeLaunch {
  double* T2;
  const double* T;
  const double* iCp;
  int64_t nx, ny;
  const Rect* rects;
  int nrects;
  StencilCoef k;
  int chunk_rows, remap;
  hipStream_t stream;
  uint64_t* sig = nullptr;
  int sig_rects = 0;
  int sig_chunk_rows = 0;
  const DirectStores* direct = nullptr;
  int* occupancy = nullptr;
  int uniform = 0;
  double c0 = 0.0;
};

template <int K, int S, int V, int Ar, int C = 1, bool WithUni = false>
void launch(const PipeLaunch& a) {
  if (a.occupancy) {
    const int bs = kWave * S * C;
    a.occupancy[0] = a.occupancy[1] = 0;
    RMA_HIP_CHECK(hipOccupancyMaxActiveBlocksPerMultiprocessor(
        &a.occupancy[0], pipe_kernel<K, S, V, Ar, C, false>, bs, 0));
    if constexpr (has_direct<V, Ar, C>())
      RMA_HIP_CHECK(hipOccupancyMaxActiveBlocksPerMultiprocessor(
          &a.occupancy[1], pipe_kernel<K, S, V, Ar, C, true>, bs, 0));
    return;
  }
  int rows_buf[kMaxRects] = {};
  const int* rows = nullptr;
  if (a.sig_rects > 0 && a.sig_chunk_rows > 0) {
    for (int i = 0; i < a.sig_rects && i < kMaxRects; ++i) rows_buf[i] = a.sig_chunk_rows;
    rows = rows_buf;
  }
  RectList L;
  const int64_t blocks =
      plan_strip_tasks(L, a.rects, a.nrects, V, a.chunk_rows, K, Geo<K, S, V, C>::WB, rows);
  static_assert(Geo<K, S, V, C>::kStep == (Geo<K, S, V, C>::WB - 2 * K) / V * V, "strip step");
  if (L.n == 0) return;
  RMA_CHECK_ARG(blocks < (int64_t(1) << 31), "grid too large: " << blocks << " blocks");
  if (a.sig) {
    int ns = 0;
    for (int i = 0; i < a.sig_rects; ++i) ns += a.rects[i].empty() ? 0 : 1;
    RMA_CHECK_ARG(ns > 0, "signalling launch without a non-empty signal rect");
    L.sig = a.sig;
    L.sig_blocks = L.block_end[ns - 1];
  }
  const dim3 grid((unsigned)blocks), block(kWave * S * C);
  if (a.direct && a.direct->on) {
    if constexpr (has_direct<V, Ar, C>()) {
      pipe_kernel<K, S, V, Ar, C, true><<<grid, block, 0, a.stream>>>(
          a.T2, a.T, a.iCp, a.nx, a.ny, L, a.k, a.chunk_rows, a.remap, *a.direct, 0.0);
    } else {
      RMA_CHECK_ARG(false, "no direct-store variant of the pipelined kernel K=" << K << " S=" << S
                                << " V=" << V << " arithmetic " << Ar << " columns " << C);
    }
    return;
  }
  if constexpr (WithUni && has_uniform<V, Ar, C>()) {
    if (a.uniform) {
      pipe_kernel<K, S, V, Ar, C, false, true><<<grid, block, 0, a.stream>>>(
          a.T2, a.T, a.iCp, a.nx, a.ny, L, a.k, a.chunk_rows, a.remap, DirectStores{}, a.c0);
      return;
    }
  }
  pipe_kernel<K, S, V, Ar, C><<<grid, block, 0, a.stream>>>(
      a.T2, a.T, a.iCp, a.nx, a.ny, L, a.k, a.chunk_rows, a.remap, DirectStores{}, 0.0);
}

bool dispatch_a(int K, int S, int V, int ar, const PipeLaunch& a);
bool dispatch_b(int K, int S, int V, int ar, const PipeLaunch& a);
bool dispatch_c(int K, int S, int V, int ar, const PipeLaunch& a);
bool dispatch_r(int K, int S, int V, int ar, const PipeLaunch& a);
bool dispatch_r20(int K, int S, int V, int ar, const PipeLaunch& a);
bool dispatch_r24(int K, int S, int V, int ar, const PipeLaunch& a);

}
}

#define RMA_PIPE_CASE(KK, SS, CC)                                  \
  if (K == KK && S == SS && ar == CC) {                            \
    if (V == 4) launch<KK, SS, 4, CC>(a);                          \
    else if (V == 2) launch<KK, SS, 2, CC>(a);                     \
    else launch<KK, SS, 1, CC>(a);                                 \
    return true;                                                   \
  }

#define RMA_PIPE_CASE_U(KK, SS, CC)                                \
  if (K == KK && S == SS && ar == CC) {                            \
    if (V == 4) launch<KK, SS, 4, CC, 1, true>(a);                 \
    else if (V == 2) launch<KK, SS, 2, CC, 1, true>(a);            \
    else launch<KK, SS, 1, CC>(a);                                 \
    return true;                                                   \
  }
```

csrc/kernels/stencil_pipe.hip:

```cpp
#include <hip/hip_runtime.h>

#include <cmath>

#include "rma/hip_check.h"
#include "rma/kernels.h"
#include "lab_hooks.h"
#include "stencil_pipe.h"

namespace rma {


void stencil_pipe_occupancy(int K, int stages, int arith, int V, int occ[2]) {
  const int S = stages > 0 ? stages : pipe_default_stages(K);
  RMA_CHECK_ARG(pipe_has(K, S, arith), "no pipelined kernel for K=" << K << " S=" << S
                                                                   << " arithmetic " << arith);
  pipe::PipeLaunch a{nullptr, nullptr, nullptr, 0, 0, nullptr, 0, StencilCoef{}, 1, 0, nullptr};
  a.occupancy = occ;
  occ[0] = occ[1] = 0;
  if (V != 5)
    (void)(pipe::dispatch_r20(K, S, V, arith, a) || pipe::dispatch_r24(K, S, V, arith, a) ||
           pipe::dispatch_r(K, S, V, arith, a) ||
           pipe::dispatch_a(K, S, V, arith, a) ||
           pipe::dispatch_b(K, S, V, arith, a) || pipe::dispatch_c(K, S, V, arith, a));
}

void stencil_pipe_rects_gpu(int K, int stages, int arith, double* T2, const double* T,
                            const double* iCp, int64_t nx, int64_t ny, const Rect* rects,
                            int nrects, const StencilCoef& c, const StencilTuning& tune,
                            stream_t stream) {
  const int S = stages > 0 ? stages : pipe_default_stages(K);
  RMA_CHECK_ARG(K >= 1 && K <= kPipeMaxK,
                "pipelined K-step kernel: 1 <= K <= " << kPipeMaxK << ", got " << K);
  RMA_CHECK_ARG(pipe_has(K, S, arith), "no pipelined kernel instantiated for K=" << K << " S=" << S
                                                                             << " arithmetic " << arith);
  const bool canonical = arith == pipe::kArCanon;
  RMA_CHECK_ARG(canonical || fast5_ok(c),
                "the fast5 arithmetic folds dy^-2/dx^-2 into one factor: needs lam != 0 and "
                "finite coefficients");
  RMA_CHECK_ARG(nrects >= 0 && nrects <= kMaxRects, "nrects=" << nrects);
  RMA_CHECK_ARG(nx >= 3 && ny >= 3, "grid too small: nx=" << nx << " ny=" << ny);
  RMA_CHECK_ARG(ny < (int64_t(1) << 30), "rows are indexed in 32 bits, ny = " << ny);
  RMA_CHECK_ARG(T2 != T, "multi-step kernel cannot run in place");
  RMA_CHECK_ARG(tune.chunk_rows >= 1, "chunk_rows=" << tune.chunk_rows);
  for (int i = 0; i < nrects; ++i) {
    const Rect& r = rects[i];
    if (r.empty()) continue;
    RMA_CHECK_ARG(r.x0 >= 1 && r.x1 <= nx - 1 && r.y0 >= 1 && r.y1 <= ny - 1,
                  "rect " << i << " outside the interior of " << nx << "x" << ny);
  }
  const bool aligned = ((reinterpret_cast<uintptr_t>(T) & 15) == 0) &&
                       ((reinterpret_cast<uintptr_t>(T2) & 15) == 0) &&
                       ((reinterpret_cast<uintptr_t>(iCp) & 15) == 0);
  const int V = pipe_vec(K, S, arith, nx, tune.vec, aligned);
  int C = tune.cols > 0 ? tune.cols : pipe_default_cols(K, S, arith);
  RMA_CHECK_ARG(pipe_has_cols(K, S, arith, C), "no pipelined kernel with " << C
                                                   << " column waves for K=" << K << " S=" << S
                                                   << " arithmetic " << arith);
  if (V != 4) C = 1;
  const int remap = tune.xcd_remap >= 0 ? tune.xcd_remap : (nx > 65536 ? 1 : 0);
  pipe::PipeLaunch a{T2, T, iCp, nx, ny, rects, nrects, c, tune.chunk_rows, remap,
                     as_stream(stream)};
  if (tune.direct && tune.direct->on) {
    const DirectStores& D = *tune.direct;
    auto inside = [](int64_t a0, int64_t a1, int64_t shift, int64_t n) {
      return a0 >= a1 || (a0 + shift >= 0 && a1 + shift <= n);
    };
    RMA_CHECK_ARG(inside(D.xm0, D.xm1, D.sx, nx) && inside(D.xp0, D.xp1, -D.sx, nx) &&
                      inside(D.ym0, D.ym1, D.syr, ny) && inside(D.yp0, D.yp1, -D.syr, ny),
                  "direct-store ranges map outside the " << nx << "x" << ny << " tile");
    for (int d = 0; d < 8; ++d) {
      if (!D.dst[d]) continue;
      RMA_CHECK_ARG(V < 2 || (D.sx % 2 == 0 && (D.syr * nx) % 2 == 0 &&
                              (reinterpret_cast<uintptr_t>(D.dst[d]) & 15) == 0),
                    "direct store " << d << ": 16-byte stores need even shifts and an aligned "
                                       "destination");
    }
    a.direct = &D;
  }
  if (tune.uniform && !a.direct) {
    a.uniform = 1;
    a.c0 = tune.uniform_value;
  }
  if (tune.signal || tune.signal_rects > 0) {
    RMA_CHECK_ARG(tune.signal_rects >= 1 && tune.signal_rects < nrects,
                  "signal rects " << tune.signal_rects << " of " << nrects);
    a.sig = tune.signal;
    a.sig_rects = tune.signal_rects;
    RMA_CHECK_ARG(tune.signal_chunk_rows >= 0, "signal_chunk_rows=" << tune.signal_chunk_rows);
    a.sig_chunk_rows = tune.signal_chunk_rows;
  }
  bool ok = C == 1 && V != 5 &&
            (pipe::dispatch_r20(K, S, V, arith, a) || pipe::dispatch_r24(K, S, V, arith, a) ||
           pipe::dispatch_r(K, S, V, arith, a) ||
             pipe::dispatch_a(K, S, V, arith, a) ||
             pipe::dispatch_b(K, S, V, arith, a) || pipe::dispatch_c(K, S, V, arith, a));
  if (!ok) {
    if (!lab_hooks().pipe)
      lab_missing("this pipelined kernel variant (stages / arithmetic / cols / 5 cells per lane)");
    ok = lab_hooks().pipe(K, S, V, C, arith, a);
  }
  RMA_CHECK_ARG(ok, "pipelined kernel K=" << K << " S=" << S << " V=" << V << " C=" << C
                                           << " arithmetic=" << arith << " not instantiated");
  RMA_HIP_LAUNCH_CHECK();
}

}
```

csrc/kernels/stencil_pipe_r.hip:

```cpp
#include "stencil_pipe.h"

namespace rma {
namespace pipe {

bool dispatch_r(int K, int S, int V, int ar, const PipeLaunch& a) {
  if (ar != kArFast5Reg) return false;
  RMA_PIPE_CASE_U(10, 4, kArFast5Reg)
  RMA_PIPE_CASE_U(11, 4, kArFast5Reg)
  RMA_PIPE_CASE_U(12, 4, kArFast5Reg)
  RMA_PIPE_CASE_U(13, 4, kArFast5Reg)
  RMA_PIPE_CASE_U(14, 4, kArFast5Reg)
  RMA_PIPE_CASE_U(15, 4, kArFast5Reg)
  RMA_PIPE_CASE_U(16, 4, kArFast5Reg)
  RMA_PIPE_CASE_U(17, 4, kArFast5Reg)
  RMA_PIPE_CASE_U(18, 4, kArFast5Reg)
  RMA_PIPE_CASE_U(19, 4, kArFast5Reg)
  RMA_PIPE_CASE_U(21, 4, kArFast5Reg)
  RMA_PIPE_CASE_U(22, 4, kArFast5Reg)
  RMA_PIPE_CASE_U(23, 4, kArFast5Reg)
  RMA_PIPE_CASE_U(24, 4, kArFast5Reg)
  return false;
}

}
}
```

csrc/kernels/stencil_pipe_r20.hip:

```cpp
#include "stencil_pipe.h"

namespace rma {
namespace pipe {

bool dispatch_r20(int K, int S, int V, int ar, const PipeLaunch& a) {
  if (ar != kArFast5Reg) return false;
  RMA_PIPE_CASE_U(20, 4, kArFast5Reg)
  return false;
}

}
}
```

csrc/kernels/stencil_pipe_r24.hip:

```cpp
#include "stencil_pipe.h"

namespace rma {
namespace pipe {

bool dispatch_r24(int K, int S, int V, int ar, const PipeLaunch& a) {
  if (ar != kArFast5RegNoSB) return false;
  RMA_PIPE_CASE_U(24, 4, kArFast5RegNoSB)
  return false;
}

}
}
```

csrc/runtime/config.cpp:

```cpp
#include "rma/config.h"

#include <cerrno>
#include <cmath>
#include <cstdlib>
#include <cstring>
#include <sstream>
#include <vector>

#include "rma/common.h"

namespace rma {

const char* const kDiagKeys[] = {
    "skip_exchange",
    "exec_streams",
    "exec_verbose",
    "no_prime",
    "no_lag",
    "no_halo_cross",
    "no_halo_merged",
    "no_halo_batch",
    "frame_sides",
    "frame_chunk_div",
    "frame_aligned",
    "frame_bands",
    "no_frame_fill",
    "pipe_fast",
    "pass_costs",
    "uniform_factor",
    "rccl_data_blocking",
    "rccl_graph",
    "no_ipc_graph",
    "hostname",
    "rccl_fallback",
    "bench_rc_dir",
    "bench_n1_cache",
    "bench_check_raise",
    "bench_check_corrupt",
    "bench_window_corrupt",
    "bench_field_corrupt",
    "bench_rccl_log_dir",
    nullptr};

namespace {

bool known(const std::string& k) {
  for (const char* const* p = kDiagKeys; *p; ++p)
    if (k == *p) return true;
  return false;
}

std::vector<std::pair<std::string, std::string>> entries() {
  std::vector<std::pair<std::string, std::string>> out;
  const char* e = std::getenv("RMA_DIAG");
  if (!e || !*e) return out;
  std::stringstream ss(e);
  std::string item;
  while (std::getline(ss, item, ',')) {
    if (item.empty()) continue;
    const size_t eq = item.find('=');
    std::string k = item.substr(0, eq), v = eq == std::string::npos ? "1" : item.substr(eq + 1);
    if (!known(k)) {
      std::string all;
      for (const char* const* p = kDiagKeys; *p; ++p) all += std::string(all.empty() ? "" : " ") + *p;
      throw_error("RMA_DIAG: unknown key", __FILE__, __LINE__, k + " (known: " + all + ")");
    }
    out.emplace_back(std::move(k), std::move(v));
  }
  return out;
}

}

std::string diag_string() {
  (void)entries();
  const char* e = std::getenv("RMA_DIAG");
  return e ? e : "";
}

bool diag_flag(const char* key) {
  for (const auto& kv : entries())
    if (kv.first == key) return kv.second != "0";
  return false;
}

std::string diag_value(const char* key, const std::string& dflt) {
  for (const auto& kv : entries())
    if (kv.first == key) return kv.second;
  return dflt;
}

double env_double(const char* name, double dflt, double lo, double hi) {
  const char* e = std::getenv(name);
  if (!e || !*e) return dflt;
  errno = 0;
  char* end = nullptr;
  const double v = std::strtod(e, &end);
  if (errno || end == e || *end != '\0' || !std::isfinite(v) || v < lo || v > hi) {
    std::ostringstream m;
    m << e << " (expected a number in [" << lo << ", " << hi << "])";
    throw_error((std::string(name) + ": bad value").c_str(), __FILE__, __LINE__, m.str());
  }
  return v;
}

std::string env_choice(const char* name, const char* choices, const char* dflt) {
  const char* e = std::getenv(name);
  if (!e || !*e) return dflt;
  std::stringstream ss(choices);
  std::string c;
  while (std::getline(ss, c, '|'))
    if (c == e) return c;
  throw_error((std::string(name) + ": bad value").c_str(), __FILE__, __LINE__,
              std::string(e) + " (one of " + choices + ")");
}

}
```

csrc/runtime/executor.cpp:

```cpp
#include "rma/executor.h"

#include <hip/hip_runtime.h>

#include <algorithm>
#include <array>
#include <chrono>
#include <cmath>
#include <cstdio>
#include <cstdlib>
#include <cstring>
#include <limits>
#include <mutex>
#include <string>
#include <thread>
#include <utility>

#include "rma/config.h"
#include "rma/hip_check.h"
#include "rma/trace.h"

namespace rma {

namespace {
hipStream_t S(void* p) { return reinterpret_cast<hipStream_t>(p); }
hipEvent_t E(void* p) { return reinterpret_cast<hipEvent_t>(p); }

std::mutex g_pool_mu;
std::vector<std::pair<hipStream_t, hipStream_t>> g_pool;
}

StencilTuning default_tune_k(int K, int64_t ny) {
  StencilTuning t;
  t.nontemporal = 3;
  if (K <= 2) {
    t.chunk_rows = 16;
    t.unroll = 2;
    return t;
  }
  t.kernel = 3;
  t.xcd_remap = 1;
  if (ny < 3072) t.chunk_rows = 16;
  else if (ny < 6144) t.chunk_rows = 32;
  else if (ny < 12288) t.chunk_rows = 64;
  else if (ny < 32768) t.chunk_rows = K <= 8 ? (K == 8 ? 128 : 256) : 256;
  else if (K >= 20 && ny >= 98304) t.chunk_rows = 3072;
  else if (K >= 12 && ny >= 98304) t.chunk_rows = 1536;
  else t.chunk_rows = K >= 8 ? 1024 : 512;
  return t;
}

StencilTuning fast_tune_k(int K, int64_t ny, const StencilCoef& c) {
  StencilTuning t = default_tune_k(std::max(K, 3), ny);
  t.xcd_remap = 1;
  if (!fast5_ok(c)) return canonical_tune_k(K, ny);
  t.kernel = 9;
  t.vec = 4;
  if (const int ch = pipe_chunk_rows(K, ny, false)) t.chunk_rows = ch;
  if ((K >= 14 || (K >= 10 && ny >= 65536)) && pipe_has(K, pipe_default_stages(K), 3))
    t.kernel = 12;
  if (K == 24 && t.kernel == 12) t.kernel = 22;
  static const std::string force = diag_value("pipe_fast");
  RMA_CHECK_ARG(force.empty() || force == "pipe" || force == "pipe5",
                "RMA_DIAG pipe_fast=" << force << " (pipe | pipe5)");
  if (force == "pipe" || force == "pipe5") t.kernel = 9;
  if (force == "pipe5") t.vec = 5;
  return t;
}

StencilTuning canonical_tune_k(int K, int64_t ny) {
  StencilTuning t = default_tune_k(K, ny);
  if (K >= 5) {
    t.kernel = 10;
    t.vec = 4;
    if (const int ch = pipe_chunk_rows(K, ny, true)) t.chunk_rows = ch;
  }
  return t;
}

DiffusionExecutor::DiffusionExecutor(double* T, double* T2, const double* iCp, int64_t nx,
                                     int64_t ny, const ExecParams& p, HaloExchanger* halo,
                                     double* qx, double* qy, double* dTdt)
    : T_(T), T2_(T2), iCp_(iCp), nx_(nx), ny_(ny), p_(p), halo_(halo), qx_(qx), qy_(qy),
      dTdt_(dTdt) {
  RMA_CHECK_ARG(nx >= 3 && ny >= 3, "grid too small: " << nx << "x" << ny);
  RMA_CHECK_ARG(T && iCp, "null field");
  RMA_CHECK_ARG(p.mode == Mode::kKp || T2 != nullptr, "T2 required");
  RMA_CHECK_ARG(p.mode != Mode::kKp || (qx && qy && dTdt), "kp needs qx, qy, dTdt");
  RMA_CHECK_ARG(!p.use_graph || !halo || halo->capturable(),
                "hipGraph replay needs a capturable halo transport (RCCL or none); the loopback "
                "transport synchronises on the host");
  RMA_CHECK_ARG(p.temporal >= 1 && p.temporal <= kPipeMaxK,
                "temporal (max steps per pass) must be 1.." << kPipeMaxK << ", got " << p.temporal);
  RMA_CHECK_ARG(p.temporal == 1 || p.mode != Mode::kKp,
                "temporal blocking applies to perf / perf_hide, not kp");
  RMA_CHECK_ARG(p.olx >= 2 && p.oly >= 2, "overlaps must be >= 2");
  RMA_CHECK_ARG(p.temporal == 1 || ny < (int64_t(1) << 30),
                "K-step passes index rows in 32 bits, ny = " << ny);
  hwx_ = hwy_ = p.temporal;
  if (halo) nbr_ = halo->neighbors();
  real_nbr_ = nbr_;
  const int64_t ol[2] = {p.olx, p.oly};
  for (int d = 0; d < 2; ++d)
    RMA_CHECK_ARG((nbr_[d][0] < 0 && nbr_[d][1] < 0) || ol[d] >= 2 * p.temporal,
                  "temporal=" << p.temporal << " needs a grid overlap >= " << 2 * p.temporal
                              << " along dim " << d << " (init_global_grid overlaps=2K, "
                              << "halowidths=K), got " << ol[d]);
  full_ = {1, nx - 1, 1, ny - 1};
  if (p.mode == Mode::kHide) {
    RMA_CHECK_ARG(p.bwx >= 1 && p.bwy >= 1,
                  "b_width must be >= 1 so the send planes belong to the boundary kernel");
    const int64_t fx = std::max(p.bwx, p.olx - 1), fy = std::max(p.bwy, p.oly - 1);
    const auto side = frame_sides(nbr_);
    split_rect_sides(full_, side[0][0] ? fx : 0, side[0][1] ? fx : 0, side[1][0] ? fy : 0,
                     side[1][1] ? fy : 0, frame_, interior_);
  } else {
    interior_ = full_;
  }
  if (p.temporal > 1 || fast5()) {
    cost_ = default_pass_costs(p.temporal, fast5(), (double)nx * (double)ny);
    {
      std::string pc = diag_value("pass_costs");
      for (char& ch : pc)
        if (ch == '/') ch = ',';
      apply_cost_overrides(cost_, pc.empty() ? nullptr : pc.c_str());
    }
    geom_.resize(p.temporal + 1);
    geom_ok_.assign(p.temporal + 1, 0);
    (void)geometry(p.temporal);
  }
  try {
  int least = 0, greatest = 0;
  RMA_HIP_CHECK(hipDeviceGetStreamPriorityRange(&least, &greatest));
  hipStream_t hi, lo;
  const std::string mode = diag_value("exec_streams", "pool");
  RMA_CHECK_ARG(mode == "pool" || mode == "lofirst" || mode == "hifirst" || mode == "plain",
                "RMA_DIAG exec_streams=" << mode << " (pool | lofirst | hifirst | plain)");
  if (mode == "pool") {
    std::lock_guard<std::mutex> lk(g_pool_mu);
    if (!g_pool.empty()) {
      lo = g_pool.back().first;
      hi = g_pool.back().second;
      g_pool.pop_back();
    } else {
      RMA_HIP_CHECK(hipStreamCreateWithPriority(&lo, hipStreamNonBlocking, least));
      RMA_HIP_CHECK(hipStreamCreateWithPriority(&hi, hipStreamNonBlocking, greatest));
    }
    pooled_ = true;
  } else if (mode == "plain") {
    RMA_HIP_CHECK(hipStreamCreateWithFlags(&lo, hipStreamNonBlocking));
    RMA_HIP_CHECK(hipStreamCreateWithFlags(&hi, hipStreamNonBlocking));
  } else if (mode == "hifirst") {
    RMA_HIP_CHECK(hipStreamCreateWithPriority(&hi, hipStreamNonBlocking, greatest));
    RMA_HIP_CHECK(hipStreamCreateWithPriority(&lo, hipStreamNonBlocking, least));
  } else {
    RMA_HIP_CHECK(hipStreamCreateWithPriority(&lo, hipStreamNonBlocking, least));
    RMA_HIP_CHECK(hipStreamCreateWithPriority(&hi, hipStreamNonBlocking, greatest));
  }
  if (diag_flag("exec_verbose"))
    fprintf(stderr, "[executor] priority range least=%d greatest=%d mode=%s hi=%p lo=%p\n", least,
            greatest, mode.c_str(), (void*)hi, (void*)lo);
  s_hi_ = hi;
  s_lo_ = lo;
  for (void** e : {&e_hi_, &e_lo_, &e_in_, &e_fr_})
    RMA_HIP_CHECK(hipEventCreateWithFlags(reinterpret_cast<hipEvent_t*>(e), hipEventDisableTiming));
  lag_ = !diag_flag("no_lag");
  const std::string fu = env_choice("RMA_EXEC_FUSED", "auto|0|1", "auto");
  fused_ = fu == "auto" ? 2 : fu == "1" ? 1 : 0;
  fused_timeout_s_ = env_double("RMA_EXEC_FUSED_TIMEOUT", 60.0, 1e-9, 1e6);
  {
    int dev = 0, cus = 0;
    RMA_HIP_CHECK(hipGetDevice(&dev));
    RMA_HIP_CHECK(hipDeviceGetAttribute(&cus, hipDeviceAttributeMultiprocessorCount, dev));
    cus_ = cus > 0 ? cus : 256;
  }
    if (fused_ && p_.mode == Mode::kHide) {
      RMA_HIP_CHECK(hipMalloc(reinterpret_cast<void**>(&sig_), 2 * sizeof(uint64_t)));
      RMA_HIP_CHECK(hipMemsetAsync(sig_, 0, 2 * sizeof(uint64_t), S(s_lo_)));
      RMA_HIP_CHECK(hipStreamSynchronize(S(s_lo_)));
      RMA_HIP_CHECK(hipHostMalloc(reinterpret_cast<void**>(&ferr_host_), sizeof(uint32_t),
                                  hipHostMallocMapped));
      *ferr_host_ = 0;
      RMA_HIP_CHECK(
          hipHostGetDevicePointer(reinterpret_cast<void**>(&ferr_dev_), ferr_host_, 0));
    }
    scan_factor();
    if (!diag_flag("no_prime")) prime();
  } catch (...) {
    release_resources();
    throw;
  }
}

DiffusionExecutor::~DiffusionExecutor() { release_resources(); }

void DiffusionExecutor::release_resources() {
  release_timing();
  if (graph_exec_) (void)hipGraphExecDestroy(reinterpret_cast<hipGraphExec_t>(graph_exec_));
  graph_exec_ = nullptr;
  for (void** e : {&e_hi_, &e_lo_, &e_in_, &e_fr_}) {
    if (*e) (void)hipEventDestroy(E(*e));
    *e = nullptr;
  }
  if (sig_ || ferr_host_) {
    if (s_hi_) (void)hipStreamSynchronize(S(s_hi_));
    if (s_lo_) (void)hipStreamSynchronize(S(s_lo_));
    if (sig_) (void)hipFree(sig_);
    if (ferr_host_) (void)hipHostFree(ferr_host_);
    sig_ = nullptr;
    ferr_host_ = nullptr;
    ferr_dev_ = nullptr;
  }
  if (!s_hi_ && !s_lo_) return;
  if (pooled_) {
    (void)hipStreamSynchronize(S(s_hi_));
    (void)hipStreamSynchronize(S(s_lo_));
    std::lock_guard<std::mutex> lk(g_pool_mu);
    g_pool.emplace_back(S(s_lo_), S(s_hi_));
  } else {
    if (s_hi_) (void)hipStreamDestroy(S(s_hi_));
    if (s_lo_) (void)hipStreamDestroy(S(s_lo_));
  }
  s_hi_ = s_lo_ = nullptr;
}

void DiffusionExecutor::scan_factor() {
  uniform_ = false;
  c0_ = 0.0;
  const std::string v = diag_value("uniform_factor");
  RMA_CHECK_ARG(v.empty() || v == "off", "RMA_DIAG uniform_factor=" << v << " (off)");
  if (v == "off" || !fast5()) return;
  RMA_HIP_CHECK(hipDeviceSynchronize());
  uint64_t* d = nullptr;
  RMA_HIP_CHECK(hipMalloc(reinterpret_cast<void**>(&d), 2 * sizeof(uint64_t)));
  uint64_t h[2] = {1, 0};
  try {
    RMA_HIP_CHECK(hipMemsetAsync(d, 0, 2 * sizeof(uint64_t), S(s_lo_)));
    count_differing_gpu(iCp_, nx_ * ny_, d, s_lo_);
    RMA_HIP_CHECK(hipMemcpyAsync(h, d, sizeof h, hipMemcpyDeviceToHost, S(s_lo_)));
    RMA_HIP_CHECK(hipStreamSynchronize(S(s_lo_)));
  } catch (...) {
    (void)hipStreamSynchronize(S(s_lo_));
    (void)hipFree(d);
    throw;
  }
  RMA_HIP_CHECK(hipFree(d));
  if (h[0] != 0) return;
  uniform_ = true;
  std::memcpy(&c0_, &h[1], sizeof c0_);
}

bool DiffusionExecutor::rescan_factor() {
  RMA_HIP_CHECK(hipStreamSynchronize(S(s_hi_)));
  RMA_HIP_CHECK(hipStreamSynchronize(S(s_lo_)));
  const bool was = uniform_;
  const double c0 = c0_;
  scan_factor();
  if ((was != uniform_ || std::memcmp(&c0, &c0_, sizeof c0) != 0) && graph_exec_) {
    (void)hipGraphExecDestroy(reinterpret_cast<hipGraphExec_t>(graph_exec_));
    graph_exec_ = nullptr;
  }
  return uniform_;
}

bool DiffusionExecutor::fast5() const {
  return p_.fast_math && p_.mode != Mode::kKp && fast5_ok(p_.coef);
}

const PassGeom& DiffusionExecutor::geometry(int K) {
  RMA_CHECK_ARG(K >= 1 && K < (int)geom_.size(), "pass depth " << K);
  if (!geom_ok_[K]) {
    const StencilTuning t = pass_tuning(K, 0);
    int64_t tw = 0, th = 0;
    int vec = t.vec;
    if (t.kernel >= 9) {
      vec = pipe_vec(K, t.stages, t.kernel - 9, nx_, t.vec, true);
      tw = (64 * vec - 2 * K) / vec * vec;
      th = t.chunk_rows;
    }
    geom_[K] = pass_geometry(nx_, ny_, K, nbr_, p_.mode == Mode::kHide, p_.bwx, p_.bwy, p_.olx,
                             p_.oly, tw, th, vec, frame_layout(ny_, nbr_).bands,
                             direct_active() ? (int)std::max(hwx_, hwy_) : 0);
    geom_[K].task_w = tw;
    geom_[K].task_h = th;
    geom_ok_[K] = 1;
  }
  return geom_[K];
}

std::vector<int> DiffusionExecutor::plan(int64_t nsteps) const {
  if (p_.mode == Mode::kKp || cost_.empty()) return std::vector<int>((size_t)nsteps, 1);
  return plan_passes(nsteps, cost_);
}

StencilTuning DiffusionExecutor::pass_tuning(int K, int part) const {
  StencilTuning t = fast5() ? fast_tune_k(K, ny_, p_.coef) : canonical_tune_k(K, ny_);
  t.nontemporal = p_.tune2.nontemporal;
  if (p_.chunk_rows2 > 0) t.chunk_rows = p_.chunk_rows2;
  if (K == 2 && !fast5()) t.unroll = p_.tune2.unroll;
  if (part == 0) return t;
  if (t.kernel >= 9 && part == 1) {
    return t;
  }
  t.chunk_rows = std::min(t.chunk_rows, 64);
  if (t.kernel >= 6) t.vec = std::min(t.vec, 2);
  return t;
}

int DiffusionExecutor::frame_chunk_rows(int K, int interior_rows) const {
  (void)K;
  return std::max(1, interior_rows / frame_layout(ny_, nbr_).chunk_div);
}

void DiffusionExecutor::exchange(double* A, stream_t s) {
  if (!halo_ || solo_) return;
  static const bool skip = [] {
    const bool on = diag_flag("skip_exchange");
    if (on)
      fprintf(stderr, "[rocm_mpi_amd] WARNING: RMA_DIAG skip_exchange: every halo exchange is "
                      "skipped, multi-rank results are WRONG (diagnosis only)\n");
    return on;
  }();
  if (skip) return;
  HaloField f;
  f.ptr = A;
  f.size = {nx_, ny_, 1};
  f.elem_bytes = 8;
  f.ol = {p_.olx, p_.oly, 2};
  f.hw = {hwx_, hwy_, 1};
  static const bool cross_ok = !diag_flag("no_halo_cross");
  static const bool merged_ok = !diag_flag("no_halo_merged");
  const bool xy = (nbr_[0][0] >= 0 || nbr_[0][1] >= 0) && (nbr_[1][0] >= 0 || nbr_[1][1] >= 0);
  if (cross_ok && cross_pass_ && p_.temporal == 1 && p_.mode != Mode::kKp)
    halo_->exchange_cross({f}, s, 3);
  else if (merged_ok && xy && halo_->has_diagonals())
    halo_->exchange_merged({f}, s);
  else
    halo_->exchange({f}, s, 3);
}

void DiffusionExecutor::enqueue_step(double* Tin, double* Tout) {
  const StencilCoef& c = p_.coef;
  if (p_.mode == Mode::kKp) {
    TraceRange tr("rma.step.kp");
    flux_gpu(qx_, qy_, Tin, nx_, ny_, c.mlam, c.rdx, c.rdy, s_lo_);
    residual_gpu(dTdt_, qx_, qy_, iCp_, nx_, ny_, c.rdx, c.rdy, s_lo_);
    update_gpu(Tin, dTdt_, nx_, ny_, c.dt, s_lo_);
    exchange(Tin, s_lo_);
    return;
  }
  void* ev[5] = {nullptr, nullptr, nullptr, nullptr, nullptr};
  if (timing_) {
    for (auto& e : ev) e = tevent();
    if (ev[4]) tk_.push_back(1);
  }
  auto rec = [&](int i, void* stream) {
    if (ev[4]) RMA_HIP_CHECK(hipEventRecord(E(ev[i]), S(stream)));
  };
  if (p_.mode == Mode::kPerf || solo_) {
    TraceRange tr("rma.step.perf");
    if (p_.mode == Mode::kHide) {
      RMA_HIP_CHECK(hipStreamWaitEvent(S(s_lo_), E(e_hi_), 0));
    }
    rec(0, s_lo_);
    rec(3, s_lo_);
    stencil_rects_gpu(Tout, Tin, iCp_, nx_, ny_, &full_, 1, c, p_.tune, s_lo_);
    rec(4, s_lo_);
    rec(1, s_lo_);
    exchange(Tout, s_lo_);
    rec(2, s_lo_);
    if (ev[4]) tseq_.push_back(1);
    if (p_.mode == Mode::kHide) RMA_HIP_CHECK(hipEventRecord(E(e_lo_), S(s_lo_)));
    return;
  }
  TraceRange tr("rma.step.hide");
  RMA_HIP_CHECK(hipStreamWaitEvent(S(s_hi_), E(e_lo_), 0));
  RMA_HIP_CHECK(hipStreamWaitEvent(S(s_lo_), E(lag_ ? e_fr_ : e_hi_), 0));
  const bool interior_first = halo_ && !halo_->capturable();
  auto interior = [&]() {
    rec(3, s_lo_);
    if (!interior_.empty()) {
      TraceRange ti("rma.interior");
      stencil_rects_gpu(Tout, Tin, iCp_, nx_, ny_, &interior_, 1, c, p_.tune, s_lo_);
    }
    rec(4, s_lo_);
    RMA_HIP_CHECK(hipEventRecord(E(e_lo_), S(s_lo_)));
  };
  if (interior_first) interior();
  rec(0, s_hi_);
  StencilTuning ft = p_.tune;
  ft.chunk_rows = std::min(ft.chunk_rows, 16);
  if (!frame_.empty()) {
    TraceRange tb("rma.boundary");
    stencil_rects_gpu(Tout, Tin, iCp_, nx_, ny_, frame_.data(), (int)frame_.size(), c, ft, s_hi_);
  }
  RMA_HIP_CHECK(hipEventRecord(E(e_fr_), S(s_hi_)));
  rec(1, s_hi_);
  {
    TraceRange th("rma.halo");
    exchange(Tout, s_hi_);
  }
  rec(2, s_hi_);
  RMA_HIP_CHECK(hipEventRecord(E(e_hi_), S(s_hi_)));
  if (!interior_first) interior();
  if (ev[4]) tseq_.push_back(0);
}

void DiffusionExecutor::multi_step(int K, double* Tin, double* Tout, const double* iCp,
                                   int64_t nx, int64_t ny, const Rect* rects, int n,
                                   const StencilTuning& tn, void* stream) const {
  if (K == 2 && tn.kernel < 5) {
    stencil2_rects_gpu(Tout, Tin, iCp, nx, ny, rects, n, p_.coef, tn, stream);
    return;
  }
  if (!uniform_) {
    stencilk_rects_gpu(K, Tout, Tin, iCp, nx, ny, rects, n, p_.coef, tn, stream);
    return;
  }
  StencilTuning tu = tn;
  tu.uniform = true;
  tu.uniform_value = c0_;
  stencilk_rects_gpu(K, Tout, Tin, iCp, nx, ny, rects, n, p_.coef, tu, stream);
}

bool DiffusionExecutor::fused_pass_ok(const PassGeom& g, const StencilTuning& tn) const {
  if (!sig_ || !g.aligned || tn.kernel < 9 || g.interior.empty()) return false;
  int nf = 0;
  for (const Rect& r : g.frame) nf += r.empty() ? 0 : 1;
  if (nf == 0 || (int)g.frame.size() + 1 > kMaxRects) return false;
  return fused_ == 1 || g.tasks() > 2 * (int64_t)cus_;
}

template <typename Launch>
void DiffusionExecutor::enqueue_fused(const std::vector<Rect>& frame, const Rect& interior,
                                      StencilTuning tn, double* Tout, void* const* ev,
                                      Launch&& launch) {
  ++fused_passes_;
  auto rec = [&](int i, void* stream) {
    if (ev[4]) RMA_HIP_CHECK(hipEventRecord(E(ev[i]), S(stream)));
  };
  RMA_HIP_CHECK(hipStreamWaitEvent(S(s_lo_), E(e_hi_), 0));
  const bool dr = direct_remote();
  if (dr) direct_wait(direct_pass_, s_lo_);
  Rect rs[kMaxRects];
  int n = 0;
  for (const Rect& r : frame) rs[n++] = r;
  tn.signal = sig_;
  tn.signal_rects = n;
  rs[n++] = interior;
  rec(0, s_hi_);
  rec(3, s_lo_);
  {
    TraceRange ti("rma.fused");
    launch(rs, n, tn);
  }
  rec(4, s_lo_);
  RMA_HIP_CHECK(hipEventRecord(E(e_lo_), S(s_lo_)));
  flag_wait_gpu(sig_ + 1, 1, fused_timeout_s_, ferr_dev_, 1, s_hi_);
  flag_write_gpu(sig_ + 1, 0, s_hi_);
  RMA_HIP_CHECK(hipEventRecord(E(e_fr_), S(s_hi_)));
  rec(1, s_hi_);
  {
    TraceRange th("rma.halo");
    if (dr)
      flags_write_gpu(dout_, direct_pass_ + 1, s_hi_);
    else
      exchange(Tout, s_hi_);
  }
  rec(2, s_hi_);
  RMA_HIP_CHECK(hipEventRecord(E(e_hi_), S(s_hi_)));
  if (ev[4]) tseq_.push_back(0);
}

void DiffusionExecutor::check_fused_error() const {
  if (!ferr_host_) return;
  const uint32_t e = __atomic_load_n(ferr_host_, __ATOMIC_ACQUIRE);
  RMA_CHECK_ARG(e != 1, "frame-first fused pass: the exchange stream's wait for the frame tasks "
                        "timed out after "
                            << fused_timeout_s_
                            << " s (RMA_EXEC_FUSED_TIMEOUT); the halos of that pass are wrong");
  RMA_CHECK_ARG(e == 0, "direct-store halos: the wait for a neighbour's pass count timed out "
                        "after "
                            << fused_timeout_s_
                            << " s (RMA_EXEC_FUSED_TIMEOUT; a neighbour died or runs another "
                               "plan); the halos of that pass are wrong");
}

void DiffusionExecutor::ensure_error_word() {
  if (ferr_host_) return;
  RMA_HIP_CHECK(hipHostMalloc(reinterpret_cast<void**>(&ferr_host_), sizeof(uint32_t),
                              hipHostMallocMapped));
  *ferr_host_ = 0;
  RMA_HIP_CHECK(hipHostGetDevicePointer(reinterpret_cast<void**>(&ferr_dev_), ferr_host_, 0));
}

void DiffusionExecutor::direct_wait(uint64_t want, void* stream) {
  if (!dhost_) {
    flags_wait_ge_gpu(din_flags_, din_mask_, want, fused_timeout_s_, ferr_dev_, 2, stream);
    return;
  }
  const auto t0 = std::chrono::steady_clock::now();
  for (int d = 0; d < 8; ++d) {
    if (!((din_mask_ >> d) & 1u)) continue;
    while (__atomic_load_n(din_flags_ + d, __ATOMIC_ACQUIRE) < want) {
      const double dt =
          std::chrono::duration<double>(std::chrono::steady_clock::now() - t0).count();
      RMA_CHECK_ARG(dt < fused_timeout_s_,
                    "direct-store halos: the host wait for the pass count of direction "
                        << d << " timed out after " << fused_timeout_s_
                        << " s (RMA_EXEC_FUSED_TIMEOUT; a neighbour died or runs another plan)");
      std::this_thread::yield();
    }
  }
}

void DiffusionExecutor::set_direct(const std::array<DirectPeer, 8>& peers, uint64_t* in_flags,
                                   bool host_wait) {
  RMA_HIP_CHECK(hipStreamSynchronize(S(s_hi_)));
  RMA_HIP_CHECK(hipStreamSynchronize(S(s_lo_)));
  bool any = false;
  uint32_t mask = 0;
  FlagTargets out{};
  const auto& nb = real_nbr_;
  const bool diag = halo_ && halo_->has_diagonals();
  for (int d = 0; d < 8; ++d) {
    const int i = kDirI[d], j = kDirJ[d];
    int want = -1;
    if (j == 0)
      want = nb[0][i > 0];
    else if (i == 0)
      want = nb[1][j > 0];
    else if (nb[0][i > 0] >= 0 && nb[1][j > 0] >= 0) {
      RMA_CHECK_ARG(diag, "direct-store halos with x and y neighbours need the diagonal ranks");
      want = halo_->diagonals()[(j > 0) * 2 + (i > 0)];
    }
    const DirectPeer& p = peers[d];
    RMA_CHECK_ARG(p.rank == want, "direct-store peer of direction (" << i << "," << j << "): rank "
                                      << p.rank << ", the grid's neighbour is " << want);
    if (p.rank < 0) continue;
    any = true;
    RMA_CHECK_ARG(p.T && p.T2, "direct-store peer (" << i << "," << j << "): null fields");
    if (p.T == T_) {
      RMA_CHECK_ARG(p.T2 == T2_, "direct-store self peer with another T2");
      continue;
    }
    RMA_CHECK_ARG(p.flag, "direct-store peer (" << i << "," << j << "): null pass-count word");
    mask |= 1u << d;
    out.dst[d] = p.flag;
    if (host_wait)
      RMA_HIP_CHECK(hipHostGetDevicePointer(reinterpret_cast<void**>(&out.dst[d]), p.flag, 0));
  }
  if (any) {
    RMA_CHECK_ARG(nx_ < (int64_t(1) << 30) && ny_ < (int64_t(1) << 30),
                  "direct-store halos: 32-bit image ranges");
    RMA_CHECK_ARG(p_.mode != Mode::kKp && fast5(),
                  "direct-store halos need fast-math K-step passes (pipelined kernels at every "
                  "depth)");
    RMA_CHECK_ARG(mask == 0 || in_flags, "direct-store halos with another rank need in_flags");
    ensure_error_word();
  }
  dpeer_ = peers;
  if (cost_base_.empty()) cost_base_ = cost_;
  cost_ = cost_base_;
  if (any) {
    const bool al = ((reinterpret_cast<uintptr_t>(T_) | reinterpret_cast<uintptr_t>(T2_) |
                      reinterpret_cast<uintptr_t>(iCp_)) & 15) == 0;
    for (int K = 1; K < (int)cost_.size(); ++K) {
      if (!std::isfinite(cost_[K])) continue;
      const StencilTuning t = pass_tuning(K, 0);
      if (t.kernel < 9) {
        cost_[K] = std::numeric_limits<double>::infinity();
        continue;
      }
      const int arith = t.kernel - 9;
      const int S = t.stages > 0 ? t.stages : pipe_default_stages(K);
      int occ[2] = {0, 0};
      stencil_pipe_occupancy(K, S, arith, pipe_vec(K, S, arith, nx_, t.vec, al), occ);
      if (occ[1] <= 0)
        cost_[K] = std::numeric_limits<double>::infinity();
      else if (occ[1] < occ[0])
        cost_[K] *= (double)occ[0] / occ[1];
    }
  }
  if (any) {
    dstores_[0] = direct_stores(false);
    dstores_[1] = direct_stores(true);
  }
  din_flags_ = in_flags;
  dhost_ = host_wait;
  din_mask_ = any ? mask : 0;
  dout_ = any ? out : FlagTargets{};
  direct_on_ = any;
  direct_pass_ = 0;
  std::fill(geom_ok_.begin(), geom_ok_.end(), 0);
  if (graph_exec_) {
    (void)hipGraphExecDestroy(reinterpret_cast<hipGraphExec_t>(graph_exec_));
    graph_exec_ = nullptr;
  }
}

bool DiffusionExecutor::images_in_frame(const PassGeom& g) const {
  const DirectStores& D = dstores_[0];
  const Rect& o = g.out;
  auto clip = [&](Rect r) {
    r.x0 = std::max(r.x0, o.x0), r.x1 = std::min(r.x1, o.x1);
    r.y0 = std::max(r.y0, o.y0), r.y1 = std::min(r.y1, o.y1);
    return r;
  };
  auto area = [](const Rect& r) { return r.empty() ? 0 : (r.x1 - r.x0) * (r.y1 - r.y0); };
  bool side[4] = {false, false, false, false};
  for (int d = 0; d < 8; ++d) {
    if (!dstores_[0].dst[d]) continue;
    if (kDirI[d] < 0) side[0] = true;
    if (kDirI[d] > 0) side[1] = true;
    if (kDirJ[d] < 0) side[2] = true;
    if (kDirJ[d] > 0) side[3] = true;
  }
  const Rect strips[4] = {{D.xm0, D.xm1, o.y0, o.y1}, {D.xp0, D.xp1, o.y0, o.y1},
                          {o.x0, o.x1, D.ym0, D.ym1}, {o.x0, o.x1, D.yp0, D.yp1}};
  for (int k = 0; k < 4; ++k) {
    if (!side[k]) continue;
    const Rect st = clip(strips[k]);
    int64_t in = 0;
    for (const Rect& f : g.frame) {
      Rect c = st;
      c.x0 = std::max(c.x0, f.x0), c.x1 = std::min(c.x1, f.x1);
      c.y0 = std::max(c.y0, f.y0), c.y1 = std::min(c.y1, f.y1);
      in += area(c);
    }
    if (in != area(st)) return false;
  }
  return true;
}

DirectStores DiffusionExecutor::direct_stores(bool out_is_T2) const {
  DirectStores D;
  D.xm0 = (int32_t)(p_.olx - hwx_);
  D.xm1 = (int32_t)p_.olx;
  D.xp0 = (int32_t)(nx_ - p_.olx);
  D.xp1 = (int32_t)(nx_ - p_.olx + hwx_);
  D.ym0 = (int32_t)(p_.oly - hwy_);
  D.ym1 = (int32_t)p_.oly;
  D.yp0 = (int32_t)(ny_ - p_.oly);
  D.yp1 = (int32_t)(ny_ - p_.oly + hwy_);
  D.sx = nx_ - p_.olx;
  D.syr = ny_ - p_.oly;
  for (int d = 0; d < 8; ++d) {
    const DirectPeer& p = dpeer_[d];
    if (p.rank < 0) continue;
    D.dst[d] = out_is_T2 ? p.T2 : p.T;
    D.on = 1;
  }
  return D;
}

void DiffusionExecutor::enqueue_pass(int K, double* Tin, double* Tout) {
  const PassGeom& g = geometry(K);
  const bool dr = direct_remote();
  const bool da = direct_active() && (dr || g.tasks() <= 2 * (int64_t)cus_);
  struct DirectCount {
    uint64_t& n;
    bool on;
    ~DirectCount() {
      if (on) ++n;
    }
  } dcount{direct_pass_, da};
  StencilTuning tn = pass_tuning(K, 0);
  auto with_direct = [&](StencilTuning t) {
    if (da) t.direct = &dstores_[Tout == T2_ ? 1 : 0];
    return t;
  };
  const StencilTuning tin = da && !images_in_frame(g) ? with_direct(tn) : tn;
  auto dwait = [&](void* stream) {
    if (dr) direct_wait(direct_pass_, stream);
  };
  auto dpost = [&](void* stream) {
    if (dr) flags_write_gpu(dout_, direct_pass_ + 1, stream);
  };
  void* ev[5] = {nullptr, nullptr, nullptr, nullptr, nullptr};
  if (timing_) {
    for (auto& e : ev) e = tevent();
    if (ev[4]) tk_.push_back(K);
  }
  auto rec = [&](int i, void* stream) {
    if (ev[4]) RMA_HIP_CHECK(hipEventRecord(E(ev[i]), S(stream)));
  };
  if (p_.mode == Mode::kPerf) {
    TraceRange tr("rma.pass.perf");
    rec(0, s_lo_);
    rec(3, s_lo_);
    dwait(s_lo_);
    multi_step(K, Tin, Tout, iCp_, nx_, ny_, &g.out, 1, with_direct(tn), s_lo_);
    rec(4, s_lo_);
    rec(1, s_lo_);
    if (da)
      dpost(s_lo_);
    else
      exchange(Tout, s_lo_);
    rec(2, s_lo_);
    if (ev[4]) tseq_.push_back(1);
    return;
  }
  if (da && (!dr || g.frame.empty() || g.tasks() <= 2 * (int64_t)cus_)) {
    TraceRange tr("rma.pass.direct");
    RMA_HIP_CHECK(hipStreamWaitEvent(S(s_lo_), E(e_hi_), 0));
    rec(0, s_lo_);
    rec(3, s_lo_);
    dwait(s_lo_);
    if (g.aligned && !g.interior.empty() && g.frame.size() + 1 <= (size_t)kMaxRects) {
      Rect rs[kMaxRects];
      int n = 0;
      for (const Rect& r : g.frame) rs[n++] = r;
      rs[n++] = g.interior;
      StencilTuning t = with_direct(tn);
      t.signal_rects = n - 1;
      t.signal_chunk_rows = frame_chunk_rows(K, tn.chunk_rows);
      multi_step(K, Tin, Tout, iCp_, nx_, ny_, rs, n, t, s_lo_);
    } else {
      multi_step(K, Tin, Tout, iCp_, nx_, ny_, &g.out, 1, with_direct(tn), s_lo_);
    }
    rec(4, s_lo_);
    rec(1, s_lo_);
    dpost(s_lo_);
    rec(2, s_lo_);
    RMA_HIP_CHECK(hipEventRecord(E(e_lo_), S(s_lo_)));
    if (ev[4]) tseq_.push_back(1);
    return;
  }
  if (g.frame.empty()) {
    TraceRange tr("rma.pass.hide");
    RMA_HIP_CHECK(hipStreamWaitEvent(S(s_lo_), E(e_hi_), 0));
    rec(0, s_lo_);
    rec(3, s_lo_);
    multi_step(K, Tin, Tout, iCp_, nx_, ny_, &g.interior, 1, tn, s_lo_);
    rec(4, s_lo_);
    rec(1, s_lo_);
    exchange(Tout, s_lo_);
    rec(2, s_lo_);
    RMA_HIP_CHECK(hipEventRecord(E(e_lo_), S(s_lo_)));
    if (ev[4]) tseq_.push_back(1);
    return;
  }
  if (fused_pass_ok(g, tn)) {
    TraceRange tr("rma.pass.fused");
    enqueue_fused(g.frame, g.interior, with_direct(tn), Tout, ev,
                  [&](const Rect* rs, int n, const StencilTuning& t) {
                    multi_step(K, Tin, Tout, iCp_, nx_, ny_, rs, n, t, s_lo_);
                  });
    return;
  }
  TraceRange tr("rma.pass.hide");
  RMA_HIP_CHECK(hipStreamWaitEvent(S(s_hi_), E(e_lo_), 0));
  RMA_HIP_CHECK(hipStreamWaitEvent(S(s_lo_), E(lag_ ? e_fr_ : e_hi_), 0));
  const bool interior_first = !da && halo_ && !halo_->capturable();
  auto interior = [&]() {
    rec(3, s_lo_);
    if (!g.interior.empty()) {
      TraceRange ti("rma.interior");
      multi_step(K, Tin, Tout, iCp_, nx_, ny_, &g.interior, 1, tin, s_lo_);
    }
    rec(4, s_lo_);
    RMA_HIP_CHECK(hipEventRecord(E(e_lo_), S(s_lo_)));
  };
  if (interior_first) interior();
  rec(0, s_hi_);
  dwait(s_hi_);
  if (!g.frame.empty()) {
    TraceRange tb("rma.boundary");
    if (g.aligned) {
      StencilTuning ft = with_direct(tn);
      ft.xcd_remap = 0;
      ft.chunk_rows = frame_chunk_rows(K, tn.chunk_rows);
      multi_step(K, Tin, Tout, iCp_, nx_, ny_, g.frame.data(), (int)g.frame.size(), ft, s_hi_);
    } else {
      const StencilTuning tw = with_direct(pass_tuning(K, 1)), tt = with_direct(pass_tuning(K, 2));
      if (!g.frame_wide.empty())
        multi_step(K, Tin, Tout, iCp_, nx_, ny_, g.frame_wide.data(), (int)g.frame_wide.size(),
                   tw, s_hi_);
      if (!g.frame_tall.empty())
        multi_step(K, Tin, Tout, iCp_, nx_, ny_, g.frame_tall.data(), (int)g.frame_tall.size(),
                   tt, s_hi_);
    }
  }
  RMA_HIP_CHECK(hipEventRecord(E(e_fr_), S(s_hi_)));
  rec(1, s_hi_);
  {
    TraceRange th("rma.halo");
    if (da)
      dpost(s_hi_);
    else
      exchange(Tout, s_hi_);
  }
  rec(2, s_hi_);
  RMA_HIP_CHECK(hipEventRecord(E(e_hi_), S(s_hi_)));
  if (!interior_first) interior();
  if (ev[4]) tseq_.push_back(0);
}

void* DiffusionExecutor::tevent() {
  constexpr size_t kMaxEvents = 5 * 8192;
  if (tused_ >= kMaxEvents) return nullptr;
  if (tused_ == tev_.size()) {
    hipEvent_t e;
    RMA_HIP_CHECK(hipEventCreate(&e));
    tev_.push_back(e);
  }
  return tev_[tused_++];
}

void DiffusionExecutor::release_timing() {
  for (void* e : tev_) (void)hipEventDestroy(E(e));
  tev_.clear();
  tk_.clear();
  tseq_.clear();
  tused_ = 0;
}

void DiffusionExecutor::set_timing(bool on) {
  RMA_HIP_CHECK(hipStreamSynchronize(S(s_hi_)));
  RMA_HIP_CHECK(hipStreamSynchronize(S(s_lo_)));
  tused_ = 0;
  tk_.clear();
  tseq_.clear();
  timing_ = on;
}

std::vector<PassTiming> DiffusionExecutor::timings() {
  RMA_HIP_CHECK(hipStreamSynchronize(S(s_hi_)));
  RMA_HIP_CHECK(hipStreamSynchronize(S(s_lo_)));
  check_fused_error();
  std::vector<PassTiming> out;
  for (size_t i = 0; i < tk_.size(); ++i) {
    hipEvent_t* e = reinterpret_cast<hipEvent_t*>(&tev_[5 * i]);
    float t[5] = {0, 0, 0, 0, 0};
    for (int j = 1; j < 5; ++j) RMA_HIP_CHECK(hipEventElapsedTime(&t[j], e[0], e[j]));
    PassTiming pt;
    pt.K = tk_[i];
    pt.frame_ms = tseq_[i] ? 0.0f : t[1];
    pt.halo_ms = t[2] - t[1];
    pt.interior_ms = t[4] - t[3];
    pt.pass_ms = std::max(t[2], t[4]);
    pt.exposed_halo_ms = std::max(0.0f, t[2] - t[4]);
    out.push_back(pt);
  }
  return out;
}

void DiffusionExecutor::set_solo(bool on) {
  RMA_HIP_CHECK(hipStreamSynchronize(S(s_hi_)));
  RMA_HIP_CHECK(hipStreamSynchronize(S(s_lo_)));
  if (on == solo_) return;
  solo_ = on;
  nbr_ = on ? Neighbors{{{-1, -1}, {-1, -1}, {-1, -1}}} : real_nbr_;
  std::fill(geom_ok_.begin(), geom_ok_.end(), 0);
  if (graph_exec_) {
    (void)hipGraphExecDestroy(reinterpret_cast<hipGraphExec_t>(graph_exec_));
    graph_exec_ = nullptr;
  }
}

void DiffusionExecutor::prime() {
  if (p_.mode == Mode::kKp || (p_.temporal == 1 && !fast5())) return;
  RMA_HIP_CHECK(hipStreamSynchronize(S(s_hi_)));
  RMA_HIP_CHECK(hipStreamSynchronize(S(s_lo_)));
  const int64_t tnx = 256 + nx_ % 4, tny = 64;
  const size_t bytes = (size_t)(tnx * tny) * sizeof(double);
  double* buf = nullptr;
  RMA_HIP_CHECK(hipMalloc(&buf, 3 * bytes));
  double *a = buf, *b = buf + tnx * tny, *ic = buf + 2 * tnx * tny;
  RMA_HIP_CHECK(hipMemsetAsync(buf, 0, 3 * bytes, S(s_lo_)));
  const Rect r{1, tnx - 1, 1, tny - 1};
  try {
    for (int K = 1; K <= p_.temporal; ++K) {
      if (!std::isfinite(cost_[K])) continue;
      if (K == 1 && !fast5()) {
        stencil_rects_gpu(b, a, ic, tnx, tny, &r, 1, p_.coef, p_.tune, s_lo_);
        continue;
      }
      multi_step(K, a, b, ic, tnx, tny, &r, 1, pass_tuning(K, 0), s_lo_);
      if (sig_ && K == p_.temporal) {
        const Rect rr[2] = {Rect{1, tnx - 1, 1, 9}, Rect{1, tnx - 1, 9, tny - 1}};
        StencilTuning st = pass_tuning(K, 0);
        if (st.kernel >= 9) {
          st.signal = sig_;
          st.signal_rects = 1;
          multi_step(K, a, b, ic, tnx, tny, rr, 2, st, s_lo_);
          flag_wait_gpu(sig_ + 1, 1, fused_timeout_s_, ferr_dev_, 1, s_lo_);
          flag_write_gpu(sig_ + 1, 0, s_lo_);
        }
      }
      if (p_.mode == Mode::kHide)
        for (int part = 1; part <= 2; ++part)
          multi_step(K, a, b, ic, tnx, tny, &r, 1, pass_tuning(K, part), s_lo_);
    }
    RMA_HIP_CHECK(hipStreamSynchronize(S(s_lo_)));
  } catch (...) {
    (void)hipStreamSynchronize(S(s_lo_));
    (void)hipFree(buf);
    throw;
  }
  RMA_HIP_CHECK(hipFree(buf));
}

void DiffusionExecutor::run_eager(int64_t nsteps) {
  if (p_.mode == Mode::kKp) {
    for (int64_t i = 0; i < nsteps; ++i) {
      enqueue_step(T_, nullptr);
      ++steps_;
      ++passes_;
    }
    return;
  }
  const std::vector<int> passes =
      cost_.empty() ? std::vector<int>((size_t)nsteps, 1) : plan_passes(nsteps, cost_);
  struct ResetCross {
    bool& f;
    ~ResetCross() { f = false; }
  } reset_cross{cross_pass_};
  for (size_t pi = 0; pi < passes.size(); ++pi) {
    const int K = passes[pi];
    cross_pass_ = pi + 1 < passes.size();
    double* Tin = parity_ ? T2_ : T_;
    double* Tout = parity_ ? T_ : T2_;
    if (K == 1 && !fast5()) {
      enqueue_step(Tin, Tout);
    } else {
      enqueue_pass(K, Tin, Tout);
    }
    steps_ += K;
    ++passes_;
    parity_ ^= 1;
  }
}

void DiffusionExecutor::build_graph(int64_t steps, int reps) {
  if (graph_exec_) {
    (void)hipGraphExecDestroy(reinterpret_cast<hipGraphExec_t>(graph_exec_));
    graph_exec_ = nullptr;
  }
  if (halo_) {
    HaloField f;
    f.ptr = T_;
    f.size = {nx_, ny_, 1};
    f.elem_bytes = 8;
    f.ol = {p_.olx, p_.oly, 2};
    f.hw = {hwx_, hwy_, 1};
    halo_->prepare({f}, 3);
    if (halo_->has_diagonals()) halo_->prepare({f}, HaloExchanger::kMerged | 3);
    halo_->prepare({f}, 3);
  }
  hipStream_t lo = S(s_lo_), hi = S(s_hi_);
  const int saved_parity = parity_;
  const int64_t saved_steps = steps_, saved_passes = passes_;
  RMA_HIP_CHECK(hipStreamBeginCapture(lo, hipStreamCaptureModeThreadLocal));
  hipGraph_t g = nullptr;
  try {
    RMA_HIP_CHECK(hipEventRecord(E(e_in_), lo));
    RMA_HIP_CHECK(hipStreamWaitEvent(hi, E(e_in_), 0));
    RMA_HIP_CHECK(hipEventRecord(E(e_hi_), hi));
    RMA_HIP_CHECK(hipEventRecord(E(e_fr_), hi));
    RMA_HIP_CHECK(hipEventRecord(E(e_lo_), lo));
    for (int r = 0; r < reps; ++r) run_eager(steps);
    RMA_HIP_CHECK(hipEventRecord(E(e_hi_), hi));
    RMA_HIP_CHECK(hipStreamWaitEvent(lo, E(e_hi_), 0));
  } catch (...) {
    hipGraph_t junk = nullptr;
    (void)hipStreamEndCapture(lo, &junk);
    if (junk) (void)hipGraphDestroy(junk);
    (void)hipGetLastError();
    parity_ = saved_parity;
    steps_ = saved_steps;
    passes_ = saved_passes;
    throw;
  }
  RMA_HIP_CHECK(hipStreamEndCapture(lo, &g));
  hipGraphExec_t ge;
  RMA_HIP_CHECK(hipGraphInstantiate(&ge, g, nullptr, nullptr, 0));
  RMA_HIP_CHECK(hipGraphDestroy(g));
  graph_exec_ = ge;
  graph_len_ = steps * reps;
  parity_ = saved_parity;
  steps_ = saved_steps;
  passes_ = saved_passes;
}

void DiffusionExecutor::run(int64_t nsteps, stream_t caller_stream) {
  RMA_CHECK_ARG(nsteps >= 0, "nsteps=" << nsteps);
  check_fused_error();
  if (nsteps == 0) return;
  hipStream_t caller = S(caller_stream);
  hipStream_t lo = S(s_lo_), hi = S(s_hi_);
  RMA_HIP_CHECK(hipEventRecord(E(e_in_), caller));
  RMA_HIP_CHECK(hipStreamWaitEvent(lo, E(e_in_), 0));
  RMA_HIP_CHECK(hipStreamWaitEvent(hi, E(e_in_), 0));
  RMA_HIP_CHECK(hipEventRecord(E(e_hi_), hi));
  RMA_HIP_CHECK(hipEventRecord(E(e_fr_), hi));
  RMA_HIP_CHECK(hipEventRecord(E(e_lo_), lo));
  int64_t left = nsteps;
  if (p_.use_graph && !direct_remote()) {
    const int64_t gl = p_.graph_steps > 0 ? p_.graph_steps : 20;
    const int64_t np = (int64_t)plan(gl).size();
    const int reps = np % 2 ? 2 : 1;
    const int64_t glen = gl * reps;
    if (left >= glen) {
      if (!graph_exec_ || graph_len_ != glen) build_graph(gl, reps);
      while (left >= glen) {
        RMA_HIP_CHECK(hipGraphLaunch(reinterpret_cast<hipGraphExec_t>(graph_exec_), lo));
        steps_ += glen;
        passes_ += np * reps;
        left -= glen;
      }
      RMA_HIP_CHECK(hipEventRecord(E(e_lo_), lo));
      RMA_HIP_CHECK(hipStreamWaitEvent(hi, E(e_lo_), 0));
      RMA_HIP_CHECK(hipEventRecord(E(e_hi_), hi));
      RMA_HIP_CHECK(hipEventRecord(E(e_fr_), hi));
    }
  }
  run_eager(left);
  if (direct_remote()) direct_wait(direct_pass_, hi);
  RMA_HIP_CHECK(hipEventRecord(E(e_hi_), hi));
  RMA_HIP_CHECK(hipEventRecord(E(e_lo_), lo));
  RMA_HIP_CHECK(hipStreamWaitEvent(caller, E(e_hi_), 0));
  RMA_HIP_CHECK(hipStreamWaitEvent(caller, E(e_lo_), 0));
}

}
```

csrc/runtime/plan.cpp:

```cpp
#include "rma/config.h"
#include "rma/plan.h"

#include <algorithm>
#include <cmath>
#include <cstdlib>
#include <limits>
#include <string>

namespace rma {

void split_rect_sides(const Rect& out, int64_t xlo, int64_t xhi, int64_t ylo, int64_t yhi,
                      std::vector<Rect>& frame, Rect& interior) {
  RMA_CHECK_ARG(xlo >= 0 && xhi >= 0 && ylo >= 0 && yhi >= 0,
                "frame widths " << xlo << "," << xhi << "," << ylo << "," << yhi);
  frame.clear();
  const int64_t xi0 = out.x0 + xlo, xi1 = out.x1 - xhi;
  const int64_t yi0 = out.y0 + ylo, yi1 = out.y1 - yhi;
  if (xi0 >= xi1 || yi0 >= yi1) {
    interior = {0, 0, 0, 0};
    if (!out.empty()) frame.push_back(out);
    return;
  }
  interior = {xi0, xi1, yi0, yi1};
  if (ylo > 0) frame.push_back({out.x0, out.x1, out.y0, yi0});
  if (yhi > 0) frame.push_back({out.x0, out.x1, yi1, out.y1});
  if (xlo > 0) frame.push_back({out.x0, xi0, yi0, yi1});
  if (xhi > 0) frame.push_back({xi1, out.x1, yi0, yi1});
}

void split_rect(const Rect& out, int64_t bwx, int64_t bwy, std::vector<Rect>& frame,
                Rect& interior) {
  RMA_CHECK_ARG(bwx >= 0 && bwy >= 0, "frame widths " << bwx << "," << bwy);
  split_rect_sides(out, bwx, bwx, bwy, bwy, frame, interior);
}

std::array<std::array<bool, 2>, 2> frame_sides(const Neighbors& nbr) {
  static const bool fs_all = diag_value("frame_sides") == "all";
  const bool any = nbr[0][0] >= 0 || nbr[0][1] >= 0 || nbr[1][0] >= 0 || nbr[1][1] >= 0;
  const bool all = any && fs_all;
  std::array<std::array<bool, 2>, 2> on{};
  for (int d = 0; d < 2; ++d)
    for (int s = 0; s < 2; ++s) on[d][s] = all || nbr[d][s] >= 0;
  return on;
}

Rect owned_rect(int64_t nx, int64_t ny, int K, const Neighbors& nbr) {
  RMA_CHECK_ARG(K >= 1, "K=" << K);
  const Rect r{nbr[0][0] >= 0 ? K : 1, nx - (nbr[0][1] >= 0 ? K : 1), nbr[1][0] >= 0 ? K : 1,
               ny - (nbr[1][1] >= 0 ? K : 1)};
  RMA_CHECK_ARG(!r.empty(), "tile " << nx << "x" << ny << " too small for " << K
                                    << "-step passes");
  return r;
}

FrameLayout frame_layout(int64_t ny, const Neighbors& nbr) {
  const bool x = nbr[0][0] >= 0 || nbr[0][1] >= 0, y = nbr[1][0] >= 0 || nbr[1][1] >= 0;
  FrameLayout f;
  if (ny >= 3072 && ny < 6144) {
    f.chunk_div = 2;
    if (x && y) f.bands = 0;
  } else if (ny >= 6144 && ny < 12288 && y) {
    if (x)
      f.chunk_div = 2;
    else
      f.bands = 0;
  }
  static const std::string cd = diag_value("frame_chunk_div");
  if (!cd.empty()) f.chunk_div = std::max(1, std::atoi(cd.c_str()));
  return f;
}

PassGeom pass_geometry(int64_t nx, int64_t ny, int K, const Neighbors& nbr, bool hide,
                       int64_t bwx, int64_t bwy, int64_t olx, int64_t oly, int64_t task_w,
                       int64_t task_h, int vec, int bands, int out_k) {
  PassGeom g;
  g.out = out_k > 0 ? owned_rect(nx, ny, out_k, nbr)
          : K == 1  ? Rect{1, nx - 1, 1, ny - 1}
                    : owned_rect(nx, ny, K, nbr);
  const bool any_nbr = nbr[0][0] >= 0 || nbr[0][1] >= 0 || nbr[1][0] >= 0 || nbr[1][1] >= 0;
  const Rect& o = g.out;
  const int64_t need_x = std::max(bwx, olx - o.x0), need_y = std::max(bwy, oly - o.y0);
  static const std::string fa = diag_value("frame_aligned");
  static const std::string fb = diag_value("frame_bands");
  const bool want = fa.empty() ? true : fa[0] != '0';
  const bool task_bands = !fb.empty() ? fb[0] == 't' : bands >= 0 ? bands == 1 : task_h <= 1024;
  const int64_t band = task_bands ? task_h : need_y;
  if (want && hide && any_nbr && task_w >= need_x && task_h >= 1 && band >= need_y &&
      o.x1 - o.x0 >= 3 * task_w && o.y1 - o.y0 >= (task_bands ? 3 * task_h : 2 * band + 1)) {
    g.aligned = true;
    const auto side = frame_sides(nbr);
    const int64_t V = std::max(1, vec);
    auto floor_v = [&](int64_t a) { return a - (((a % V) + V) % V); };
    const int64_t xl = side[0][0] ? floor_v(o.x0 - K) + K + task_w : o.x0;
    int64_t xr = o.x1;
    if (side[0][1]) {
      xr = o.x1 - task_w;
      xr += ((V - ((xr - K) % V + V) % V) % V);
    }
    const int64_t yb = side[1][0] ? o.y0 + band : o.y0;
    const int64_t yt = side[1][1] ? o.y1 - band : o.y1;
    if (side[1][0]) g.frame_wide.push_back({o.x0, o.x1, o.y0, yb});
    if (side[1][1]) g.frame_wide.push_back({o.x0, o.x1, yt, o.y1});
    if (side[0][0]) g.frame_tall.push_back({o.x0, xl, yb, yt});
    if (side[0][1]) g.frame_tall.push_back({xr, o.x1, yb, yt});
    g.frame = g.frame_wide;
    g.frame.insert(g.frame.end(), g.frame_tall.begin(), g.frame_tall.end());
    g.interior = {xl, xr, yb, yt};
    return g;
  }
  if (hide && any_nbr) {
    int64_t fx = std::max(bwx, olx - g.out.x0);
    static const bool fill = !diag_flag("no_frame_fill");
    if (K >= 5 && fill)
      fx = std::max<int64_t>(fx, std::min<int64_t>(128 - 2 * K, (g.out.x1 - g.out.x0) / 4));
    const int64_t fy = std::max(bwy, oly - g.out.y0);
    const auto side = frame_sides(nbr);
    split_rect_sides(g.out, side[0][0] ? fx : 0, side[0][1] ? fx : 0, side[1][0] ? fy : 0,
                     side[1][1] ? fy : 0, g.frame, g.interior);
    for (const Rect& r : g.frame)
      (r.x1 - r.x0 >= r.y1 - r.y0 ? g.frame_wide : g.frame_tall).push_back(r);
  } else {
    g.interior = g.out;
  }
  return g;
}

namespace {
constexpr double kInf = std::numeric_limits<double>::infinity();

constexpr int kTables = 4;
constexpr double kTileCells[kTables] = {4096.0 * 4096, 8192.0 * 8192, 16384.0 * 16384,
                                        101376.0 * 101376};
constexpr double kFast5[kTables][25] = {
    {0, 1.087, 1.056, 1.102, 1.123, 1.173, 1.169, 1.207, 1.228, 1.579, 1.404, 1.355, 1.379,
     1.598, 1.638, 1.745, 1.811, 2.056, 2.170, 2.198, 2.211, 2.553, 2.575, 2.617, 2.607},
    {0, 1.530, 1.519, 1.452, 1.377, 1.487, 1.432, 1.473, 1.334, 1.823, 1.414, 1.422, 1.391,
     1.488, 1.529, 1.745, 1.782, 2.259, 2.214, 2.176, 2.182, 2.390, 2.419, 2.434, 2.283},
    {0, 1.373, 1.375, 1.412, 1.298, 1.282, 1.275, 1.273, 1.217, 1.414, 1.326, 1.328, 1.294,
     1.410, 1.440, 1.605, 1.575, 1.896, 1.922, 1.885, 1.943, 2.101, 2.119, 2.168, 2.197},
    {0, 1.235, 1.230, 1.215, 1.163, 1.232, 1.210, 1.199, 1.126, 1.149, 1.138, 1.144, 1.119,
     1.244, 1.306, 1.371, 1.399, 1.595, 1.640, 1.676, 1.658, 1.886, 1.903, 1.971, 1.962}
};
constexpr double kCanon[kTables][25] = {
    {0, 1.000, 1.058, 1.095, 1.246, 1.335, 1.326, 1.757, 1.897, 2.226, 2.214, 2.295, 2.384,
     3.189, 3.233, 3.308, 3.355, 4.007, 4.073, 4.101, 4.158, 6.194, 6.136, 6.273, 6.421},
    {0, 1.000, 1.107, 1.406, 1.375, 1.462, 1.476, 1.646, 1.596, 1.830, 1.959, 2.005, 2.095,
     2.944, 3.023, 3.038, 3.010, 3.566, 3.589, 3.593, 3.659, 5.558, 5.537, 5.664, 5.745},
    {0, 1.000, 1.124, 1.382, 1.302, 1.444, 1.436, 1.451, 1.455, 1.733, 1.867, 1.889, 1.970,
     2.784, 2.772, 2.798, 2.857, 3.333, 3.319, 3.364, 3.467, 5.660, 5.443, 5.489, 5.591},
    {0, 1.000, 1.079, 1.146, 1.067, 1.212, 1.178, 1.362, 1.398, 1.597, 1.755, 1.833, 1.885,
     2.306, 2.383, 2.491, 2.533, 2.863, 2.947, 3.079, 3.131, 4.643, 4.586, 4.713, 4.770}};
}

int pipe_chunk_rows(int K, int64_t ny, bool canonical) {
  if (ny < 1024) return 0;
  if (ny < 3072) {
    if (canonical) return K <= 6 ? 16 : K <= 8 ? 32 : 48;
    return K <= 8 ? 16 : K <= 14 ? 32 : 48;
  }
  if (ny < 6144) {
    if (canonical) return K <= 12 ? 64 : 192;
    return K <= 4 ? 32 : K <= 9 ? 64 : K <= 16 ? 128 : 192;
  }
  if (ny < 12288) {
    if (canonical) return K <= 12 ? 128 : 256;
    return K <= 9 ? 256 : K <= 16 ? 128 : 256;
  }
  if (ny < 24576) {
    if (canonical) return K <= 9 ? 256 : K <= 12 ? 512 : 384;
    return K <= 4 ? 768 : K <= 9 ? 1536 : 512;
  }
  if (ny < 32768) {
    if (K <= 9) return 0;
    return canonical ? 512 : 768;
  }
  return 0;
}

std::vector<double> default_pass_costs(int kmax, bool fast5, double cells) {
  RMA_CHECK_ARG(kmax >= 1 && kmax <= 24, "kmax=" << kmax << " (tables cover 1..24)");
  int t = kTables - 1;
  if (cells > 0) {
    double best = 1e300;
    for (int i = 0; i < kTables; ++i) {
      const double d = std::fabs(std::log(cells / kTileCells[i]));
      if (d < best) {
        best = d;
        t = i;
      }
    }
  }
  std::vector<double> c(kmax + 1, kInf);
  for (int K = 1; K <= kmax; ++K) c[K] = fast5 ? kFast5[t][K] : kCanon[t][K];
  return c;
}

void apply_cost_overrides(std::vector<double>& cost, const char* spec) {
  if (!spec || !*spec) return;
  std::string s(spec);
  size_t pos = 0;
  while (pos < s.size()) {
    size_t end = s.find(',', pos);
    if (end == std::string::npos) end = s.size();
    const std::string item = s.substr(pos, end - pos);
    const size_t colon = item.find(':');
    RMA_CHECK_ARG(colon != std::string::npos, "pass_costs item '" << item << "' is not K:cost");
    const int K = std::atoi(item.substr(0, colon).c_str());
    const double v = std::atof(item.substr(colon + 1).c_str());
    RMA_CHECK_ARG(K >= 1 && K < (int)cost.size(), "pass_costs: K=" << K << " out of range");
    RMA_CHECK_ARG(v > 0, "pass_costs: cost must be > 0 (inf disables), got " << v);
    cost[K] = v;
    pos = end + 1;
  }
}

std::vector<int> plan_passes(int64_t n, const std::vector<double>& cost) {
  RMA_CHECK_ARG(n >= 0, "n=" << n);
  const int kmax = (int)cost.size() - 1;
  RMA_CHECK_ARG(kmax >= 1, "empty cost table");
  std::vector<int> out;
  if (n == 0) return out;
  int kbest = 0;
  for (int K = 1; K <= kmax; ++K)
    if (std::isfinite(cost[K]) && (kbest == 0 || cost[K] / K < cost[kbest] / kbest)) kbest = K;
  RMA_CHECK_ARG(kbest > 0, "no pass depth available");
  int64_t rest = n;
  if (rest > 4096) {
    const int64_t q = (rest - 4096) / kbest;
    out.assign((size_t)q, kbest);
    rest -= q * kbest;
  }
  const int m = (int)rest;
  std::vector<double> best(m + 1, kInf);
  std::vector<int> pick(m + 1, 0), npass(m + 1, 0);
  best[0] = 0;
  for (int s = 1; s <= m; ++s) {
    for (int K = std::min(kmax, s); K >= 1; --K) {
      if (!std::isfinite(cost[K]) || !std::isfinite(best[s - K])) continue;
      const double v = best[s - K] + cost[K];
      const int np = npass[s - K] + 1;
      if (v < best[s] - 1e-9 || (v <= best[s] + 1e-9 && np < npass[s])) {
        best[s] = v;
        pick[s] = K;
        npass[s] = np;
      }
    }
    RMA_CHECK_ARG(pick[s] > 0, "no pass sequence covers " << s << " steps");
  }
  for (int s = m; s > 0; s -= pick[s]) out.push_back(pick[s]);
  std::sort(out.begin(), out.end(), [](int a, int b) { return a > b; });
  return out;
}

}
```

rocm_mpi_amd/config.py:

```python
from __future__ import annotations

import os

DIAG_KEYS = {
    "skip_exchange": "every halo exchange skipped (WRONG multi-rank results)",
    "exec_streams": "pool | lofirst | hifirst | plain: executor stream creation",
    "exec_verbose": "print the executor's stream priorities",
    "no_prime": "no kernel priming at executor construction",
    "no_lag": "every pass waits for the previous exchange",
    "no_halo_cross": "one-step passes: one RCCL group per dimension",
    "no_halo_merged": "x+y neighbours: one group per dimension (C++ and Python)",
    "no_halo_batch": "one pack / unpack launch per plane",
    "frame_sides": "all: frame rects on every side once any neighbour exists",
    "frame_chunk_div": "N: aligned frame tasks of 1/N the interior's rows",
    "frame_aligned": "0 | 1: force the frame layout",
    "frame_bands": "task | ol: force the aligned y-band height",
    "no_frame_fill": "frame bands not filled into the interior",
    "pipe_fast": "pipe | pipe5: the LDS-ring fast kernel at every depth",
    "pass_costs": "K:cost/K:cost/...: planner cost overrides",
    "uniform_factor": "off: the 1/Cp field path also where 1/Cp is one value",
    "rccl_data_blocking": "blocking RCCL data path of a non-blocking communicator",
    "rccl_graph": "allow hipGraph capture over RCCL",
    "no_ipc_graph": "refuse hipGraph capture over the IPC transport",
    "hostname": "node name for the local-rank exchange (tests)",
    "rccl_fallback": "an RCCL init failure falls back to the staged transport",
    "bench_rc_dir": "bench.py: every rank writes its exit status into this directory",
    "bench_n1_cache": "bench.py: path of the N = 1 record",
    "bench_check_raise": "bench.py: before | after: injected halo-check failure",
    "bench_check_corrupt": "bench.py: corrupt one halo-check cell",
    "bench_window_corrupt": "bench.py: corrupt one headline-window cell",
    "bench_field_corrupt": "bench.py: nan | hot | cold: one bad timed-field cell",
    "bench_rccl_log_dir": "bench.py: RCCL log directory of the link probe",
}


def diag_entries(s: str | None = None) -> dict:
    s = os.environ.get("RMA_DIAG", "") if s is None else s
    out = {}
    for item in filter(None, (p.strip() for p in s.split(","))):
        k, _, v = item.partition("=")
        if k not in DIAG_KEYS:
            raise ValueError(f"RMA_DIAG: unknown key {k!r} (known: {', '.join(DIAG_KEYS)})")
        out[k] = v if "=" in item else "1"
    return out


def diag_flag(key: str) -> bool:
    assert key in DIAG_KEYS, key
    v = diag_entries().get(key)
    return v is not None and v != "0"


def diag_value(key: str, default: str = "") -> str:
    assert key in DIAG_KEYS, key
    return diag_entries().get(key, default)


def diag_with(base: str | None = None, **kv) -> str:
    d = diag_entries(base)
    for k, v in kv.items():
        if k not in DIAG_KEYS:
            raise ValueError(f"unknown RMA_DIAG key {k!r}")
        if v is None or v is False:
            d.pop(k, None)
        else:
            d[k] = "1" if v is True else str(v)
    return ",".join(k if v == "1" else f"{k}={v}" for k, v in d.items())
```

Measured before the change: 86470.

## Add six-cells-per-lane uniform-factor pipe kernel and separate uniform pass cost table

Measured after the change: 94680, median of 6. +9.5%, better.

```diff
diff --git a/csrc/bindings/module.cpp b/csrc/bindings/module.cpp
--- a/csrc/bindings/module.cpp
+++ b/csrc/bindings/module.cpp
@@ -530,6 +530,8 @@
   m.def("default_chunk_k", [](int K, int64_t ny) { return default_tune_k(K, ny).chunk_rows; },
         py::arg("K"), py::arg("ny"));
   m.def("plan_passes", &plan_passes, py::arg("nsteps"), py::arg("costs"));
+  m.def("uniform_pass_costs", &uniform_pass_costs, py::arg("kmax"), py::arg("cells") = 0.0);
+  m.def("pipe_uniform_cells", &pipe_uniform_cells, py::arg("K"), py::arg("cells"));
   m.def("default_pass_costs", &default_pass_costs, py::arg("kmax"), py::arg("fast5"),
         py::arg("cells") = 0.0);
   m.def("pipe_default_stages", &pipe_default_stages, py::arg("K"));
@@ -539,6 +541,9 @@
         py::arg("cols"));
   m.def("pipe_vec", &pipe_vec, py::arg("K"), py::arg("stages"), py::arg("arith"), py::arg("nx"),
         py::arg("requested"), py::arg("aligned16") = true);
+  m.def("pipe_vec_uniform", &pipe_vec_uniform, py::arg("K"), py::arg("stages"), py::arg("arith"),
+        py::arg("nx"), py::arg("requested"), py::arg("aligned16") = true,
+        py::arg("uniform") = false);
   m.def("pipe_max_k", []() { return kPipeMaxK; });
   m.def(
       "pass_geometry",
@@ -701,6 +706,7 @@
             d["frame_tall"] = rl(g.frame_tall);
             d["interior"] = from_rect(g.interior);
             d["tasks"] = g.tasks();
+            d["task_w"] = g.task_w;
             return d;
           },
           py::arg("K"));
diff --git a/csrc/include/rma/executor.h b/csrc/include/rma/executor.h
--- a/csrc/include/rma/executor.h
+++ b/csrc/include/rma/executor.h
@@ -92,6 +92,7 @@
   void scan_factor();
   bool uniform_ = false;
   double c0_ = 0.0;
+  int cells_ = 0;
 
   double* T_;
   double* T2_;
@@ -107,6 +108,7 @@
   std::vector<char> geom_ok_;
   std::vector<double> cost_;
   std::vector<double> cost_base_;
+  std::vector<double> cost_uni_;
   int64_t hwx_ = 1, hwy_ = 1;
   void* s_hi_ = nullptr;
   void* s_lo_ = nullptr;
diff --git a/csrc/include/rma/kernels.h b/csrc/include/rma/kernels.h
--- a/csrc/include/rma/kernels.h
+++ b/csrc/include/rma/kernels.h
@@ -60,6 +60,8 @@
 bool pipe_has_cols(int K, int stages, int arith, int cols);
 int pipe_default_cols(int K, int stages, int arith);
 int pipe_vec(int K, int stages, int arith, int64_t nx, int requested, bool aligned16);
+int pipe_vec_uniform(int K, int stages, int arith, int64_t nx, int requested, bool aligned16,
+                     bool uniform);
 void stencil_pipe_occupancy(int K, int stages, int arith, int V, int occ[2]);
 void stencil_pipe_rects_gpu(int K, int stages, int arith, double* T2, const double* T,
                             const double* iCp, int64_t nx, int64_t ny, const Rect* rects,
diff --git a/csrc/include/rma/plan.h b/csrc/include/rma/plan.h
--- a/csrc/include/rma/plan.h
+++ b/csrc/include/rma/plan.h
@@ -43,6 +43,8 @@
 FrameLayout frame_layout(int64_t ny, const Neighbors& nbr);
 
 std::vector<double> default_pass_costs(int kmax, bool fast5, double cells = 0);
+std::vector<double> uniform_pass_costs(int kmax, double cells);
+int pipe_uniform_cells(int K, double cells);
 void apply_cost_overrides(std::vector<double>& cost, const char* spec);
 
 int pipe_chunk_rows(int K, int64_t ny, bool canonical);
diff --git a/csrc/kernels/kernel_select.cpp b/csrc/kernels/kernel_select.cpp
--- a/csrc/kernels/kernel_select.cpp
+++ b/csrc/kernels/kernel_select.cpp
@@ -41,6 +41,14 @@
   return 1;
 }
 
+int pipe_vec_uniform(int K, int stages, int arith, int64_t nx, int requested, bool aligned16,
+                     bool uniform) {
+  const int S = stages > 0 ? stages : pipe_default_stages(K);
+  if (requested == 6 && uniform && aligned16 && nx % 2 == 0 && pipe::pipe_has_v6(K, S, arith))
+    return 6;
+  return pipe_vec(K, stages, arith, nx, requested == 6 ? 4 : requested, aligned16);
+}
+
 int stencil_vec(int64_t nx, const StencilTuning& tune) {
   if (nx % 2) return 1;
   if (tune.vec == 4 && nx % 4 == 0) return 4;
diff --git a/csrc/kernels/pipe_arith.h b/csrc/kernels/pipe_arith.h
--- a/csrc/kernels/pipe_arith.h
+++ b/csrc/kernels/pipe_arith.h
@@ -10,5 +10,9 @@
   return ar == kArFast5 && S == 4 && K >= 16 && K <= 20;
 }
 
+inline bool pipe_has_v6(int K, int S, int ar) {
+  return S == 4 && ((ar == kArFast5Reg && K >= 17 && K <= 23) || (ar == kArFast5RegNoSB && K == 24));
+}
+
 }
 }
diff --git a/csrc/kernels/stencil_pipe.h b/csrc/kernels/stencil_pipe.h
--- a/csrc/kernels/stencil_pipe.h
+++ b/csrc/kernels/stencil_pipe.h
@@ -82,7 +82,7 @@
 template <int K, int S, int V, int Ar, int C = 1, bool Uni = false>
 constexpr int lds_bytes_reg() {
   return ((Uni ? 2 : 4) * (S > 1 ? S - 1 : 1) * Geo<K, S, V, C>::WB +
-          (V == 2 || V == 4
+          (V == 2 || V == 4 || V == 6
                ? (Uni ? 1 : 2) * staging_rows<K, S, Ar, Uni>() * Geo<K, S, V, C>::W * C
                : 0)) *
              8 +
@@ -143,11 +143,13 @@
   using P = Plan<K, S>;
   constexpr bool Canon = Ar == kArCanon, kRegG = ar_reg(Ar);
   static_assert(!kRegG || (V != 5 && (C == 1 || V == 4)),
-                "register factors: V <= 4; two column waves at V = 4 only");
-  constexpr bool kGlds = kRegG && (V == 2 || V == 4);
+                "register factors: V = 1, 2, 4 (6: uniform factor); two column waves at V = 4 "
+                "only");
+  constexpr bool kGlds = kRegG && (V == 2 || V == 4 || V == 6);
   static_assert(!Uni || (kGlds && C == 1 && !Dir),
-                "uniform factor: register factors, 2 or 4 cells per lane, one column wave, "
+                "uniform factor: register factors, 2, 4 or 6 cells per lane, one column wave, "
                 "no direct stores");
+  static_assert(V != 6 || Uni, "6 cells per lane: the uniform-factor variant only");
   constexpr bool kU6 = pipe_u6<K, S, Ar, Uni>();
   constexpr int NST = staging_rows<K, S, Ar, Uni>();
   using G = Geo<K, S, V, C>;
@@ -187,6 +189,12 @@
   const int64_t xl = min(max(x, (int64_t)0), nx - V);
   const uint32_t xo = (uint32_t)xl, xso = (uint32_t)x;
   const uint32_t xob = xo * 8u, xsob = xso * 8u;
+  uint32_t xpb[V == 6 ? 3 : 1];
+  if constexpr (V == 6) {
+#pragma unroll
+    for (int h = 0; h < 3; ++h)
+      xpb[h] = (uint32_t)min(max(x + 2 * h, (int64_t)0), nx - 2) * 8u;
+  }
   auto at = [](const double* base, uint32_t boff) {
     return reinterpret_cast<const double*>(reinterpret_cast<const char*>(base) + boff);
   };
@@ -225,7 +233,16 @@
   auto rowc = [&](int y) { return (int64_t)min(max(y, 0), ny32 - 1); };
   auto rowp = [&](const double* a, int y) { return at(a + rowc(y) * nx, xob); };
   if (stage == 0) {
-    load_row<V>(w[0][2], rowp(T, i));
+    if constexpr (V == 6) {
+#pragma unroll
+      for (int h = 0; h < 3; ++h) {
+        const dbl2 t2 = *reinterpret_cast<const dbl2*>(at(T + rowc(i) * nx, xpb[h]));
+        w[0][2][2 * h] = t2.x;
+        w[0][2][2 * h + 1] = t2.y;
+      }
+    } else {
+      load_row<V>(w[0][2], rowp(T, i));
+    }
     if constexpr (!kGlds) {
       load_row<V>(pT, rowp(T, i + 1));
       load_row<V>(pC, rowp(iCp, i));
@@ -260,7 +277,8 @@
     const double* rb = (a ? iCp : T) + rowc(y) * nx;
 #pragma unroll
     for (int h = 0; h < V / 2; ++h)
-      __builtin_amdgcn_global_load_lds(at(rb, xob + 16u * h), stg(a, r) + h * 2 * kWave, 16, 0, 0);
+      __builtin_amdgcn_global_load_lds(at(rb, V == 6 ? xpb[h] : xob + 16u * h),
+                                       stg(a, r) + h * 2 * kWave, 16, 0, 0);
   };
   if constexpr (kGlds) {
     if (stage == 0) {
@@ -432,6 +450,12 @@
           const double gu = __hiloint2double(rin ? gUhi : 0, rin ? gUlo : 0);
 #pragma unroll
           for (int v = 0; v < V; ++v) gl[v] = gu;
+        } else if constexpr (V == 6) {
+          int rz = __builtin_amdgcn_readfirstlane((int)rin);
+          asm volatile("" : "+s"(rz));
+          const double gu = __hiloint2double(rz ? gUhi : 0, rz ? gUlo : 0);
+#pragma unroll
+          for (int v = 0; v < V; ++v) gl[v] = cin[v] ? gu : 0.0;
         } else {
 #pragma unroll
           for (int v = 0; v < V; ++v) gl[v] = rin ? gc[v] : 0.0;
@@ -589,7 +613,7 @@
 
 template <int V, int Ar, int C>
 constexpr bool has_uniform() {
-  return C == 1 && (V == 2 || V == 4) && (Ar == kArFast5Reg || Ar == kArFast5RegNoSB);
+  return C == 1 && (V == 2 || V == 4 || V == 6) && (Ar == kArFast5Reg || Ar == kArFast5RegNoSB);
 }
 
 struct PipeLaunch {
@@ -616,11 +640,16 @@
   if (a.occupancy) {
     const int bs = kWave * S * C;
     a.occupancy[0] = a.occupancy[1] = 0;
-    RMA_HIP_CHECK(hipOccupancyMaxActiveBlocksPerMultiprocessor(
-        &a.occupancy[0], pipe_kernel<K, S, V, Ar, C, false>, bs, 0));
-    if constexpr (has_direct<V, Ar, C>())
+    if constexpr (V == 6) {
       RMA_HIP_CHECK(hipOccupancyMaxActiveBlocksPerMultiprocessor(
-          &a.occupancy[1], pipe_kernel<K, S, V, Ar, C, true>, bs, 0));
+          &a.occupancy[0], pipe_kernel<K, S, V, Ar, C, false, true>, bs, 0));
+    } else {
+      RMA_HIP_CHECK(hipOccupancyMaxActiveBlocksPerMultiprocessor(
+          &a.occupancy[0], pipe_kernel<K, S, V, Ar, C, false>, bs, 0));
+      if constexpr (has_direct<V, Ar, C>())
+        RMA_HIP_CHECK(hipOccupancyMaxActiveBlocksPerMultiprocessor(
+            &a.occupancy[1], pipe_kernel<K, S, V, Ar, C, true>, bs, 0));
+    }
     return;
   }
   int rows_buf[kMaxRects] = {};
@@ -643,25 +672,34 @@
     L.sig_blocks = L.block_end[ns - 1];
   }
   const dim3 grid((unsigned)blocks), block(kWave * S * C);
-  if (a.direct && a.direct->on) {
-    if constexpr (has_direct<V, Ar, C>()) {
-      pipe_kernel<K, S, V, Ar, C, true><<<grid, block, 0, a.stream>>>(
-          a.T2, a.T, a.iCp, a.nx, a.ny, L, a.k, a.chunk_rows, a.remap, *a.direct, 0.0);
-    } else {
-      RMA_CHECK_ARG(false, "no direct-store variant of the pipelined kernel K=" << K << " S=" << S
-                                << " V=" << V << " arithmetic " << Ar << " columns " << C);
-    }
-    return;
-  }
-  if constexpr (WithUni && has_uniform<V, Ar, C>()) {
-    if (a.uniform) {
-      pipe_kernel<K, S, V, Ar, C, false, true><<<grid, block, 0, a.stream>>>(
-          a.T2, a.T, a.iCp, a.nx, a.ny, L, a.k, a.chunk_rows, a.remap, DirectStores{}, a.c0);
+  if constexpr (V == 6) {
+    static_assert(WithUni && has_uniform<V, Ar, C>(), "6 cells per lane: uniform factor");
+    RMA_CHECK_ARG(a.uniform && !(a.direct && a.direct->on),
+                  "6 cells per lane without a uniform 1/Cp or with direct-store halos");
+    pipe_kernel<K, S, V, Ar, C, false, true><<<grid, block, 0, a.stream>>>(
+        a.T2, a.T, a.iCp, a.nx, a.ny, L, a.k, a.chunk_rows, a.remap, DirectStores{}, a.c0);
+  } else {
+    if (a.direct && a.direct->on) {
+      if constexpr (has_direct<V, Ar, C>()) {
+        pipe_kernel<K, S, V, Ar, C, true><<<grid, block, 0, a.stream>>>(
+            a.T2, a.T, a.iCp, a.nx, a.ny, L, a.k, a.chunk_rows, a.remap, *a.direct, 0.0);
+      } else {
+        RMA_CHECK_ARG(false, "no direct-store variant of the pipelined kernel K="
+                                 << K << " S=" << S << " V=" << V << " arithmetic " << Ar
+                                 << " columns " << C);
+      }
       return;
     }
-  }
-  pipe_kernel<K, S, V, Ar, C><<<grid, block, 0, a.stream>>>(
-      a.T2, a.T, a.iCp, a.nx, a.ny, L, a.k, a.chunk_rows, a.remap, DirectStores{}, 0.0);
+    if constexpr (WithUni && has_uniform<V, Ar, C>()) {
+      if (a.uniform) {
+        pipe_kernel<K, S, V, Ar, C, false, true><<<grid, block, 0, a.stream>>>(
+            a.T2, a.T, a.iCp, a.nx, a.ny, L, a.k, a.chunk_rows, a.remap, DirectStores{}, a.c0);
+        return;
+      }
+    }
+    pipe_kernel<K, S, V, Ar, C><<<grid, block, 0, a.stream>>>(
+        a.T2, a.T, a.iCp, a.nx, a.ny, L, a.k, a.chunk_rows, a.remap, DirectStores{}, 0.0);
+  }
 }
 
 bool dispatch_a(int K, int S, int V, int ar, const PipeLaunch& a);
@@ -689,3 +727,10 @@
     else launch<KK, SS, 1, CC>(a);                                 \
     return true;                                                   \
   }
+
+#define RMA_PIPE_CASE_U6(KK, SS, CC)                               \
+  if (K == KK && S == SS && ar == CC && V == 6) {                  \
+    launch<KK, SS, 6, CC, 1, true>(a);                             \
+    return true;                                                   \
+  }                                                                \
+  RMA_PIPE_CASE_U(KK, SS, CC)
diff --git a/csrc/kernels/stencil_pipe.hip b/csrc/kernels/stencil_pipe.hip
--- a/csrc/kernels/stencil_pipe.hip
+++ b/csrc/kernels/stencil_pipe.hip
@@ -51,7 +51,8 @@
   const bool aligned = ((reinterpret_cast<uintptr_t>(T) & 15) == 0) &&
                        ((reinterpret_cast<uintptr_t>(T2) & 15) == 0) &&
                        ((reinterpret_cast<uintptr_t>(iCp) & 15) == 0);
-  const int V = pipe_vec(K, S, arith, nx, tune.vec, aligned);
+  const bool uni = tune.uniform && !(tune.direct && tune.direct->on);
+  const int V = pipe_vec_uniform(K, S, arith, nx, tune.vec, aligned, uni);
   int C = tune.cols > 0 ? tune.cols : pipe_default_cols(K, S, arith);
   RMA_CHECK_ARG(pipe_has_cols(K, S, arith, C), "no pipelined kernel with " << C
                                                    << " column waves for K=" << K << " S=" << S
diff --git a/csrc/kernels/stencil_pipe_r.hip b/csrc/kernels/stencil_pipe_r.hip
--- a/csrc/kernels/stencil_pipe_r.hip
+++ b/csrc/kernels/stencil_pipe_r.hip
@@ -12,12 +12,12 @@
   RMA_PIPE_CASE_U(14, 4, kArFast5Reg)
   RMA_PIPE_CASE_U(15, 4, kArFast5Reg)
   RMA_PIPE_CASE_U(16, 4, kArFast5Reg)
-  RMA_PIPE_CASE_U(17, 4, kArFast5Reg)
-  RMA_PIPE_CASE_U(18, 4, kArFast5Reg)
-  RMA_PIPE_CASE_U(19, 4, kArFast5Reg)
-  RMA_PIPE_CASE_U(21, 4, kArFast5Reg)
-  RMA_PIPE_CASE_U(22, 4, kArFast5Reg)
-  RMA_PIPE_CASE_U(23, 4, kArFast5Reg)
+  RMA_PIPE_CASE_U6(17, 4, kArFast5Reg)
+  RMA_PIPE_CASE_U6(18, 4, kArFast5Reg)
+  RMA_PIPE_CASE_U6(19, 4, kArFast5Reg)
+  RMA_PIPE_CASE_U6(21, 4, kArFast5Reg)
+  RMA_PIPE_CASE_U6(22, 4, kArFast5Reg)
+  RMA_PIPE_CASE_U6(23, 4, kArFast5Reg)
   RMA_PIPE_CASE_U(24, 4, kArFast5Reg)
   return false;
 }
diff --git a/csrc/kernels/stencil_pipe_r20.hip b/csrc/kernels/stencil_pipe_r20.hip
--- a/csrc/kernels/stencil_pipe_r20.hip
+++ b/csrc/kernels/stencil_pipe_r20.hip
@@ -5,7 +5,7 @@
 
 bool dispatch_r20(int K, int S, int V, int ar, const PipeLaunch& a) {
   if (ar != kArFast5Reg) return false;
-  RMA_PIPE_CASE_U(20, 4, kArFast5Reg)
+  RMA_PIPE_CASE_U6(20, 4, kArFast5Reg)
   return false;
 }
 
diff --git a/csrc/kernels/stencil_pipe_r24.hip b/csrc/kernels/stencil_pipe_r24.hip
--- a/csrc/kernels/stencil_pipe_r24.hip
+++ b/csrc/kernels/stencil_pipe_r24.hip
@@ -5,7 +5,7 @@
 
 bool dispatch_r24(int K, int S, int V, int ar, const PipeLaunch& a) {
   if (ar != kArFast5RegNoSB) return false;
-  RMA_PIPE_CASE_U(24, 4, kArFast5RegNoSB)
+  RMA_PIPE_CASE_U6(24, 4, kArFast5RegNoSB)
   return false;
 }
 
diff --git a/csrc/runtime/config.cpp b/csrc/runtime/config.cpp
--- a/csrc/runtime/config.cpp
+++ b/csrc/runtime/config.cpp
@@ -28,6 +28,7 @@
     "pipe_fast",
     "pass_costs",
     "uniform_factor",
+    "pipe_cells",
     "rccl_data_blocking",
     "rccl_graph",
     "no_ipc_graph",
diff --git a/csrc/runtime/executor.cpp b/csrc/runtime/executor.cpp
--- a/csrc/runtime/executor.cpp
+++ b/csrc/runtime/executor.cpp
@@ -123,6 +123,9 @@
       for (char& ch : pc)
         if (ch == '/') ch = ',';
       apply_cost_overrides(cost_, pc.empty() ? nullptr : pc.c_str());
+      cost_base_ = cost_;
+      cost_uni_ = fast5() ? uniform_pass_costs(p.temporal, (double)nx * (double)ny) : cost_;
+      apply_cost_overrides(cost_uni_, pc.empty() ? nullptr : pc.c_str());
     }
     geom_.resize(p.temporal + 1);
     geom_ok_.assign(p.temporal + 1, 0);
@@ -226,6 +229,12 @@
 void DiffusionExecutor::scan_factor() {
   uniform_ = false;
   c0_ = 0.0;
+  std::fill(geom_ok_.begin(), geom_ok_.end(), 0);
+  if (!cost_base_.empty() && !direct_on_) cost_ = cost_base_;
+  const std::string cells = diag_value("pipe_cells");
+  RMA_CHECK_ARG(cells.empty() || cells == "4" || cells == "6",
+                "RMA_DIAG pipe_cells=" << cells << " (4 | 6)");
+  cells_ = cells.empty() ? 0 : cells == "4" ? 4 : 6;
   const std::string v = diag_value("uniform_factor");
   RMA_CHECK_ARG(v.empty() || v == "off", "RMA_DIAG uniform_factor=" << v << " (off)");
   if (v == "off" || !fast5()) return;
@@ -247,6 +256,7 @@
   if (h[0] != 0) return;
   uniform_ = true;
   std::memcpy(&c0_, &h[1], sizeof c0_);
+  if (!cost_base_.empty() && !direct_on_) cost_ = cost_uni_;
 }
 
 bool DiffusionExecutor::rescan_factor() {
@@ -273,7 +283,8 @@
     int64_t tw = 0, th = 0;
     int vec = t.vec;
     if (t.kernel >= 9) {
-      vec = pipe_vec(K, t.stages, t.kernel - 9, nx_, t.vec, true);
+      vec = pipe_vec_uniform(K, t.stages, t.kernel - 9, nx_, t.vec, true,
+                             uniform_ && !direct_active());
       tw = (64 * vec - 2 * K) / vec * vec;
       th = t.chunk_rows;
     }
@@ -297,6 +308,9 @@
   t.nontemporal = p_.tune2.nontemporal;
   if (p_.chunk_rows2 > 0) t.chunk_rows = p_.chunk_rows2;
   if (K == 2 && !fast5()) t.unroll = p_.tune2.unroll;
+  const bool six =
+      cells_ == 6 || (cells_ == 0 && pipe_uniform_cells(K, (double)nx_ * (double)ny_) == 6);
+  if (uniform_ && !direct_active() && six && (t.kernel == 12 || t.kernel == 22)) t.vec = 6;
   if (part == 0) return t;
   if (t.kernel >= 9 && part == 1) {
     return t;
@@ -560,7 +574,7 @@
   }
   dpeer_ = peers;
   if (cost_base_.empty()) cost_base_ = cost_;
-  cost_ = cost_base_;
+  cost_ = uniform_ && !any && !cost_uni_.empty() ? cost_uni_ : cost_base_;
   if (any) {
     const bool al = ((reinterpret_cast<uintptr_t>(T_) | reinterpret_cast<uintptr_t>(T2_) |
                       reinterpret_cast<uintptr_t>(iCp_)) & 15) == 0;
diff --git a/csrc/runtime/plan.cpp b/csrc/runtime/plan.cpp
--- a/csrc/runtime/plan.cpp
+++ b/csrc/runtime/plan.cpp
@@ -150,6 +150,23 @@
      2.784, 2.772, 2.798, 2.857, 3.333, 3.319, 3.364, 3.467, 5.660, 5.443, 5.489, 5.591},
     {0, 1.000, 1.079, 1.146, 1.067, 1.212, 1.178, 1.362, 1.398, 1.597, 1.755, 1.833, 1.885,
      2.306, 2.383, 2.491, 2.533, 2.863, 2.947, 3.079, 3.131, 4.643, 4.586, 4.713, 4.770}};
+
+constexpr double kUniformCells = 98304.0 * 98304.0;
+constexpr double kUniform288[25] = {
+    0, 1.235, 1.230, 1.215, 1.163, 1.232, 1.210, 1.199, 1.126, 1.149, 0.903, 0.902, 0.905,
+    1.138, 1.079, 1.117, 1.142, 1.273, 1.280, 1.327, 1.399, 1.459, 1.505, 1.527, 1.546};
+}
+
+int pipe_uniform_cells(int K, double cells) {
+  return cells >= kUniformCells && K >= 17 && K <= 24 ? 6 : 4;
+}
+
+std::vector<double> uniform_pass_costs(int kmax, double cells) {
+  if (cells < kUniformCells) return default_pass_costs(kmax, true, cells);
+  RMA_CHECK_ARG(kmax >= 1 && kmax <= 24, "kmax=" << kmax << " (tables cover 1..24)");
+  std::vector<double> c(kmax + 1, kInf);
+  for (int K = 1; K <= kmax; ++K) c[K] = kUniform288[K];
+  return c;
 }
 
 int pipe_chunk_rows(int K, int64_t ny, bool canonical) {
diff --git a/rocm_mpi_amd/config.py b/rocm_mpi_amd/config.py
--- a/rocm_mpi_amd/config.py
+++ b/rocm_mpi_amd/config.py
@@ -19,6 +19,7 @@
     "pipe_fast": "pipe | pipe5: the LDS-ring fast kernel at every depth",
     "pass_costs": "K:cost/K:cost/...: planner cost overrides",
     "uniform_factor": "off: the 1/Cp field path also where 1/Cp is one value",
+    "pipe_cells": "4 | 6: uniform passes at four cells everywhere / six on every tile",
     "rccl_data_blocking": "blocking RCCL data path of a non-blocking communicator",
     "rccl_graph": "allow hipGraph capture over RCCL",
     "no_ipc_graph": "refuse hipGraph capture over the IPC transport",
```
